# 2InfinityN6eyond/AbsoluteTrack

Hardware: AMD Instinct MI355X
Metric: hand-frames/sec (higher is better)
Workload: dtype f32 (backbone products as two fp16 pieces per operand, fp32 accumulation); 1 GPU; 4 fisheye cameras x 2 hands per frame, 2 views per hand, 96x96 crops, known-skeleton path, full hot path (resample+backbone+head+FK) + all-gather of records; frames_per_gpu=1024, src_image=480x636 u8 x 4 cameras, parallelism=frame-shard x1, world=1, backend=none (single process), outputs_finite=True

## Files before the change

absolutetrack_amd/csrc/conv_c32s2.hip:

```cpp
#include "ut_kernels.h"
#include "ut_conv_dev.h"

namespace ut {
namespace {

constexpr int S_OPIX = 96;
constexpr int S_PROWS = 432;
constexpr int S_STAGE = S_PROWS * 128;
constexpr int S_ZROW = 2 * S_STAGE;
constexpr int S_W8 = S_ZROW + 256;
constexpr int S_CNT = S_W8 + 2 * 4096;
constexpr int S_LDS = S_CNT + 32;
constexpr unsigned S_HOOB = 0x80000000u;
static_assert(S_ZROW % 256 == 0, "zero block bank-row aligned");

#define UT_AR_TAP_8 "v", "v", "v", "v"

}

__global__ __launch_bounds__(512, 1) void conv_c32s2_kernel(Stride2Launch p, int n_tiles) {
  extern __shared__ __attribute__((aligned(16))) char smem[];
  const unsigned smem_addr = (unsigned)(unsigned long)(lds_char*)smem;
  const int tid = threadIdx.x;
  const int lane = tid & 63;
  const int wave = __builtin_amdgcn_readfirstlane(tid >> 6);
  const bool mfma_wave = wave < 6;
  const int cb = wave & 1;
  const int blk = mfma_wave ? wave >> 1 : 0;
  const int fr = lane & 31, fh = lane >> 5;
  const int W = p.W, Wo = p.W / 2;
  const int tiles_per_img = p.H / 8;
  const int M_in = p.n_img * p.H * p.W;
  const int M_out = p.n_img * (p.H / 2) * Wo;
  constexpr int CIN = 32, COUT = 64;

  float x_scale = 1.f, x_unscale = 1.f;
  if (p.in_max) {
    bool ok, adapted;
    split_act_scale(p.in_max, p.in_obs, p.split_adaptive, x_scale, x_unscale, ok, adapted);
    split_scale_report(ok, adapted, p.status, p.adapt_count);
  }
  const float unscale1 = p.unscale1 * x_unscale, unscale_d = p.unscale_d * x_unscale;

  const u32x4 a_words = rsrc_words(p.in, (unsigned)((size_t)M_in * CIN * sizeof(float)));
  const __amdgpu_buffer_rsrc_t o1_rsrc = __builtin_amdgcn_make_buffer_rsrc(p.out1, 0, (int)((size_t)M_out * COUT * sizeof(float)), 0x00020000);
  const __amdgpu_buffer_rsrc_t o2_rsrc = __builtin_amdgcn_make_buffer_rsrc(p.out2, 0, (int)((size_t)M_out * COUT * sizeof(float)), 0x00020000);

  u32x4 wa[32], wd[4];
  {
    const char* wg = reinterpret_cast<const char*>(p.w1_split) + (size_t)cb * 9 * 4096 + lane * 16;
    asm volatile(
        "global_load_dwordx4 %0, %16, off offset:0\n\t"
        "global_load_dwordx4 %1, %16, off offset:1024\n\t"
        "global_load_dwordx4 %2, %16, off offset:2048\n\t"
        "global_load_dwordx4 %3, %16, off offset:3072\n\t"
        "global_load_dwordx4 %4, %17, off offset:0\n\t"
        "global_load_dwordx4 %5, %17, off offset:1024\n\t"
        "global_load_dwordx4 %6, %17, off offset:2048\n\t"
        "global_load_dwordx4 %7, %17, off offset:3072\n\t"
        "global_load_dwordx4 %8, %18, off offset:0\n\t"
        "global_load_dwordx4 %9, %18, off offset:1024\n\t"
        "global_load_dwordx4 %10, %18, off offset:2048\n\t"
        "global_load_dwordx4 %11, %18, off offset:3072\n\t"
        "global_load_dwordx4 %12, %19, off offset:0\n\t"
        "global_load_dwordx4 %13, %19, off offset:1024\n\t"
        "global_load_dwordx4 %14, %19, off offset:2048\n\t"
        "global_load_dwordx4 %15, %19, off offset:3072\n\t"
        "s_waitcnt vmcnt(0)"
        : "=&" UT_ARF_0(wa[0]), "=&" UT_ARF_1(wa[1]), "=&" UT_ARF_2(wa[2]), "=&" UT_ARF_3(wa[3]), "=&" UT_ARF_4(wa[4]), "=&" UT_ARF_5(wa[5]), "=&" UT_ARF_6(wa[6]), "=&" UT_ARF_7(wa[7]), "=&" UT_ARF_8(wa[8]), "=&" UT_ARF_9(wa[9]), "=&" UT_ARF_10(wa[10]), "=&" UT_ARF_11(wa[11]), "=&" UT_ARF_12(wa[12]), "=&" UT_ARF_13(wa[13]), "=&" UT_ARF_14(wa[14]), "=&" UT_ARF_15(wa[15])
        : "v"(wg + 0 * 4096), "v"(wg + 1 * 4096), "v"(wg + 2 * 4096), "v"(wg + 3 * 4096)
        : "memory");
    asm volatile(
        "global_load_dwordx4 %0, %16, off offset:0\n\t"
        "global_load_dwordx4 %1, %16, off offset:1024\n\t"
        "global_load_dwordx4 %2, %16, off offset:2048\n\t"
        "global_load_dwordx4 %3, %16, off offset:3072\n\t"
        "global_load_dwordx4 %4, %17, off offset:0\n\t"
        "global_load_dwordx4 %5, %17, off offset:1024\n\t"
        "global_load_dwordx4 %6, %17, off offset:2048\n\t"
        "global_load_dwordx4 %7, %17, off offset:3072\n\t"
        "global_load_dwordx4 %8, %18, off offset:0\n\t"
        "global_load_dwordx4 %9, %18, off offset:1024\n\t"
        "global_load_dwordx4 %10, %18, off offset:2048\n\t"
        "global_load_dwordx4 %11, %18, off offset:3072\n\t"
        "global_load_dwordx4 %12, %19, off offset:0\n\t"
        "global_load_dwordx4 %13, %19, off offset:1024\n\t"
        "global_load_dwordx4 %14, %19, off offset:2048\n\t"
        "global_load_dwordx4 %15, %19, off offset:3072\n\t"
        "s_waitcnt vmcnt(0)"
        : "=&" UT_ARF_16(wa[16]), "=&" UT_ARF_17(wa[17]), "=&" UT_ARF_18(wa[18]), "=&" UT_ARF_19(wa[19]), "=&" UT_ARF_20(wa[20]), "=&" UT_ARF_21(wa[21]), "=&" UT_ARF_22(wa[22]), "=&" UT_ARF_23(wa[23]), "=&" UT_ARF_24(wa[24]), "=&" UT_ARF_25(wa[25]), "=&" UT_ARF_26(wa[26]), "=&" UT_ARF_27(wa[27]), "=&" UT_ARF_28(wa[28]), "=&" UT_ARF_29(wa[29]), "=&" UT_ARF_30(wa[30]), "=&" UT_ARF_31(wa[31])
        : "v"(wg + 4 * 4096), "v"(wg + 5 * 4096), "v"(wg + 6 * 4096), "v"(wg + 7 * 4096)
        : "memory");
    if (wave < 2) {
#pragma unroll
      for (int q = 0; q < 4; ++q)
        *reinterpret_cast<u32x4*>(smem + S_W8 + cb * 4096 + q * 1024 + lane * 16) = *reinterpret_cast<const u32x4*>(wg + 8 * 4096 + q * 1024);
    }
    const char* dg = reinterpret_cast<const char*>(p.wd_split) + (size_t)cb * 4096 + lane * 16;
#pragma unroll
    for (int q = 0; q < 4; ++q) wd[q] = *reinterpret_cast<const u32x4*>(dg + q * 1024);
  }
  const unsigned w8 = (unsigned)(S_W8 + cb * 4096 + lane * 16);

  if (tid < 16) *reinterpret_cast<u32x4*>(smem + S_ZROW + tid * 16) = u32x4{0, 0, 0, 0};
  if (tid == 16) *reinterpret_cast<u32x4*>(smem + S_CNT) = u32x4{0, 0, 0, 0};

  const int grid = gridDim.x;
  const int my_tiles = (n_tiles - (int)blockIdx.x + grid - 1) / grid;
  const int n_pieces = (9 * W + 7) / 8;
  int lane_o = lane, wave_o = wave;
  auto patch_first_pixel = [&](int tile) {
    const int img = tile / tiles_per_img, q = tile - img * tiles_per_img;
    return img * p.H * W + (8 * q - 1) * W;
  };
  auto issue_patch_piece = [&](int i, int first_pixel, int buf) {
    const int q = wave_o + 8 * i;
    if (q < n_pieces) {
      const int pos = 8 * q + (lane_o >> 3);
      const int row = (pos & ~3) | ((pos & 1) << 1) | ((pos >> 1) & 1);
      const int pix = first_pixel + row;
      const bool ok = pix >= 0 && pix < M_in && row < 9 * W;
      const unsigned off = ok ? (unsigned)(pix * CIN + 4 * ((lane_o & 7) ^ ((row >> 2) & 7))) * 4u : S_HOOB;
      dma_piece(a_words, (unsigned)__builtin_amdgcn_readfirstlane((int)(smem_addr + (unsigned)(buf * S_STAGE + q * 1024))), off, 0u);
    }
  };
  auto convert_row = [&](int buf, int row) {
    const int sw = (row >> 2) & 7;
    char* rp = smem + buf * S_STAGE + row * 128;
    float4 f[8];
#pragma unroll
    for (int g4 = 0; g4 < 8; ++g4) f[g4] = *reinterpret_cast<const float4*>(rp + ((g4 ^ sw) << 4));
#pragma unroll
    for (int kg = 0; kg < 4; ++kg) {
      unsigned a0, a1, a2, a3, b0, b1, b2, b3;
      split_pair_scaled(f[2 * kg].x, f[2 * kg].y, x_scale, a0, b0);
      split_pair_scaled(f[2 * kg].z, f[2 * kg].w, x_scale, a1, b1);
      split_pair_scaled(f[2 * kg + 1].x, f[2 * kg + 1].y, x_scale, a2, b2);
      split_pair_scaled(f[2 * kg + 1].z, f[2 * kg + 1].w, x_scale, a3, b3);
      u32x4 a, b;
      a.x = a0; a.y = a1; a.z = a2; a.w = a3;
      b.x = b0; b.y = b1; b.z = b2; b.w = b3;
      *reinterpret_cast<u32x4*>(rp + ((kg ^ sw) << 4)) = a;
      *reinterpret_cast<u32x4*>(rp + (((4 + kg) ^ sw) << 4)) = b;
    }
  };
  auto unit_pos = [&](int u) { return (u & ~31) | (4 * ((u & 15) >> 1) + (u & 1) + 2 * ((u >> 4) & 1)); };
  auto convert_share = [&](int buf) {
    int t_ = tid;
    asm volatile("" : "+v"(t_));
    if (t_ >= 384) {
      convert_row(buf, unit_pos(t_ - 384));
      convert_row(buf, unit_pos(t_ - 384 + 128));
    } else {
      const int pos = unit_pos(256 + t_);
      if (256 + t_ < ((9 * W + 31) & ~31) && pos < 9 * W) convert_row(buf, pos);
    }
  };

  {
    const int fp = patch_first_pixel((int)blockIdx.x);
#pragma unroll
    for (int i = 0; i < 7; ++i) issue_patch_piece(i, fp, 0);
  }
  asm volatile("s_waitcnt vmcnt(0) lgkmcnt(0)" ::: "memory");
  __syncthreads();
  convert_share(0);
  __builtin_amdgcn_s_waitcnt(0xC07F);
  __builtin_amdgcn_s_barrier();

  unsigned out_bits = 0;
  const float bias1 = p.bias1[32 * cb + fr], bias_d = p.bias_d[32 * cb + fr];
  const int o_ = 32 * blk + fr, oy_ = o_ / Wo, ox_ = o_ - oy_ * Wo;
  const int lrow = 2 * oy_ * W + 2 * ox_ - 1;
  const unsigned mask_left = ox_ == 0 ? 0x1FFu & ~0x49u : 0x1FFu;
  const unsigned mask_top = oy_ == 0 ? 0x1FFu & ~0x7u : 0x1FFu;
  const unsigned cnt_addr = smem_addr + (unsigned)S_CNT;

#define S_PIN() __builtin_amdgcn_sched_barrier(0)
#define S_SIGNAL(ADDR)                                                                               \
  {                                                                                                  \
    unsigned long long keep_;                                                                        \
    asm volatile("s_mov_b64 %0, exec\n\ts_mov_b64 exec, 1\n\tds_add_u32 %1, %2\n\ts_mov_b64 exec, %0" \
                 : "=&s"(keep_) : "v"(ADDR), "v"(1u) : "memory");                                    \
  }
#define S_AWAIT(ADDR, TARGET)                                                                        \
  for (;;) {                                                                                         \
    unsigned seen_;                                                                                  \
    asm volatile("ds_read_b32 %0, %1\n\ts_waitcnt lgkmcnt(0)" : "=v"(seen_) : "v"(ADDR) : "memory"); \
    if ((int)(__builtin_amdgcn_readfirstlane(seen_) - (unsigned)(TARGET)) >= 0) break;               \
    __builtin_amdgcn_s_sleep(1);                                                                     \
  }
#define S_MFMA_A(ACC, TAP, S, PL, PXV) asm volatile("v_mfma_f32_32x32x16_f16 %0, %1, %2, %0" : "+v"(ACC) : "v"(PXV), UT_AR(TAP, S, PL)(wa[S_W(TAP, S, PL)]))
#define S_MFMA_A_FIRST(ACC, TAP, S, PL, PXV) asm volatile("s_nop 3\n\tv_mfma_f32_32x32x16_f16 %0, %1, %2, %0" : "+v"(ACC) : "v"(PXV), UT_AR(TAP, S, PL)(wa[S_W(TAP, S, PL)]))
#define S_MFMA_V(ACC, WV, PXV) asm volatile("v_mfma_f32_32x32x16_f16 %0, %1, %2, %0" : "+v"(ACC) : "v"(PXV), "v"(WV))
#define S_MFMA_V_FIRST(ACC, WV, PXV) asm volatile("s_nop 3\n\tv_mfma_f32_32x32x16_f16 %0, %1, %2, %0" : "+v"(ACC) : "v"(PXV), "v"(WV))
#define S_MFMA_V_LAST(ACC, WV, PXV) asm volatile("v_mfma_f32_32x32x16_f16 %0, %1, %2, %0\n\ts_nop 15\n\ts_nop 7" : "+v"(ACC) : "v"(PXV), "v"(WV))
#define S_W(TAP, S, PL) (((TAP) * 4 + (S) * 2 + (PL)) & 31)
#define S_ADDR(DST, BUF, TAP)                                                                        \
  {                                                                                                  \
    const int row_ = lrow_t + ((TAP) / 3) * W + ((TAP) % 3);                                         \
    const int pos_ = (row_ & ~3) | ((row_ & 1) << 1) | ((row_ >> 1) & 1);                            \
    const unsigned a_ = (unsigned)(BUF) + (unsigned)(pos_ * 128) + (unsigned)(((fh ^ ((row_ >> 2) & 7))) << 4); \
    DST = ((rmask >> (TAP)) & 1u) ? a_ : (unsigned)S_ZROW + (a_ & 255u);                             \
  }
#define S_LOAD(DST, ADDR, S)                                                                         \
  {                                                                                                  \
    DST[0] = *reinterpret_cast<const u32x4*>(smem + ((ADDR) ^ (32u * (S))));                         \
    DST[1] = *reinterpret_cast<const u32x4*>(smem + ((ADDR) ^ (32u * (S)) ^ 64u));                   \
  }
#define S_STEP(TAP, S, CUR, FAR, PIECE, ADN, ADF)                                                    \
  {                                                                                                  \
    u32x4 w8a_, w8b_;                                                                                \
    if constexpr ((TAP) == 8) {                                                                      \
      w8a_ = *reinterpret_cast<const u32x4*>(smem + w8 + ((S) * 2 + 0) * 1024);                      \
      w8b_ = *reinterpret_cast<const u32x4*>(smem + w8 + ((S) * 2 + 1) * 1024);                      \
    }                                                                                                \
    if constexpr ((TAP) < 8) {                                                                       \
      if constexpr ((TAP) == 0 && (S) == 0) { S_MFMA_A_FIRST(acc, TAP, S, 0, CUR[1]); } else { S_MFMA_A(acc, TAP, S, 0, CUR[1]); } \
    } else { S_MFMA_V(acc, w8a_, CUR[1]); }                                                          \
    S_PIN();                                                                                         \
    if constexpr ((TAP) < 8) S_LOAD(FAR, ADN, S);                                                    \
    S_PIN();                                                                                         \
    if constexpr ((TAP) < 8) { S_MFMA_A(acc, TAP, S, 1, CUR[0]); } else { S_MFMA_V(acc, w8b_, CUR[0]); } \
    S_PIN();                                                                                         \
    if constexpr ((S) == 1 && (TAP) < 7) S_ADDR(ADF, rbuf, (TAP) + 2);                               \
    S_PIN();                                                                                         \
    if constexpr ((TAP) < 8) { S_MFMA_A(acc, TAP, S, 0, CUR[0]); }                                   \
    else if constexpr ((S) == 1) { S_MFMA_V_LAST(acc, w8a_, CUR[0]); } else { S_MFMA_V(acc, w8a_, CUR[0]); } \
    S_PIN();                                                                                         \
    if constexpr ((TAP) == 4) {                     \
      if constexpr ((S) == 0) { S_MFMA_V_FIRST(accd, wd[0], CUR[1]); } else { S_MFMA_V(accd, wd[2], CUR[1]); } \
      S_PIN();                                                                                       \
      S_MFMA_V(accd, wd[2 * (S) + 1], CUR[0]); S_PIN();                                              \
      if constexpr ((S) == 1) { S_MFMA_V_LAST(accd, wd[2], CUR[0]); } else { S_MFMA_V(accd, wd[0], CUR[0]); } \
      S_PIN();                                                                                       \
    }                                                                                                \
    if ((PIECE) < 7 && dma_on) issue_patch_piece(PIECE, f_first, f_buf);                             \
    if ((PIECE) == 77 && dma_on) {       \
      asm volatile("s_waitcnt vmcnt(0)" ::: "memory");                      \
      S_SIGNAL(cnt_addr);                                                                            \
    }                                                                                                \
    S_PIN();                                                                                         \
  }

#define S_ROFF(OFF, R) ((((R) >> 3) ? (OFF) + 16u * COUT * 4u : (OFF)) + (unsigned)(((((R) >> 2) & 1) * 8 + ((R) & 3)) * COUT * 4))
#define S_EPILOGUE()                                                                                 \
  {                                                                                                  \
    const unsigned off = (unsigned)((tile * S_OPIX + 32 * blk + 4 * fh) * COUT + 32 * cb + fr) * 4u; \
    unsigned mx = 0;                                                                                 \
    _Pragma("unroll") for (int r = 0; r < 16; ++r) {                                                 \
      const float o = fmaxf(__builtin_fmaf(acc[r], unscale1, bias1), 0.f);                           \
      mx = max(mx, __float_as_uint(o));                                                              \
      __builtin_amdgcn_raw_buffer_store_b32(__float_as_uint(o), o1_rsrc, S_ROFF(off, r), 0, 0);      \
    }                                                                                                \
    out_bits = max(out_bits, mx);                                                                    \
    _Pragma("unroll") for (int r = 0; r < 16; ++r) {                                                 \
      const float o = __builtin_fmaf(accd[r], unscale_d, bias_d);                                    \
      __builtin_amdgcn_raw_buffer_store_b32(__float_as_uint(o), o2_rsrc, S_ROFF(off, r), 0, 0);      \
    }                                                                                                \
  }

  f32x16 acc, accd;
  for (int k = 0; k < my_tiles; ++k) {
    const int tile = blockIdx.x + k * grid;
    const unsigned rbuf = (unsigned)((k & 1) * S_STAGE);
    const bool dma_on = k + 1 < my_tiles;
    const int f_buf = (k + 1) & 1;
    const int f_first = patch_first_pixel(tile + grid);
    asm volatile("" : "+v"(lane_o));
    asm volatile("" : "+s"(wave_o));
    if (mfma_wave) {
      const int tq = tile % tiles_per_img;
      const unsigned rmask = mask_left & (tq == 0 ? mask_top : 0x1FFu);
      int lrow_t = lrow;
      asm volatile("" : "+v"(lrow_t));
#pragma unroll
      for (int e = 0; e < 16; ++e) { acc[e] = 0.f; accd[e] = 0.f; }
      asm volatile("" : "+v"(acc), "+v"(accd));
      {
        u32x4 pxA[2], pxB[2], pxC[2];
        unsigned adE, adO;
        S_ADDR(adE, rbuf, 0);
        S_LOAD(pxA, adE, 0);
        S_LOAD(pxB, adE, 1);
        S_ADDR(adO, rbuf, 1);
        S_STEP(0, 0, pxA, pxC, 0, adO, adE)   S_STEP(0, 1, pxB, pxA, 1, adO, adE)
        S_STEP(1, 0, pxC, pxB, 2, adE, adO)   S_STEP(1, 1, pxA, pxC, 3, adE, adO)
        S_STEP(2, 0, pxB, pxA, 4, adO, adE)   S_STEP(2, 1, pxC, pxB, 5, adO, adE)
        S_STEP(3, 0, pxA, pxC, 6, adE, adO)   S_STEP(3, 1, pxB, pxA, 99, adE, adO)
        S_STEP(4, 0, pxC, pxB, 99, adO, adE)  S_STEP(4, 1, pxA, pxC, 99, adO, adE)
        S_STEP(5, 0, pxB, pxA, 99, adE, adO)  S_STEP(5, 1, pxC, pxB, 99, adE, adO)
        S_STEP(6, 0, pxA, pxC, 99, adO, adE)  S_STEP(6, 1, pxB, pxA, 99, adO, adE)
        S_STEP(7, 0, pxC, pxB, 77, adE, adO)  S_STEP(7, 1, pxA, pxC, 99, adE, adO)
        S_STEP(8, 0, pxB, pxA, 99, adO, adE)  S_STEP(8, 1, pxC, pxB, 99, adO, adE)
      }
      asm volatile("s_nop 15\n\ts_nop 3" : "+v"(acc), "+v"(accd));
      if (wave >= 4) S_EPILOGUE();
    } else if (dma_on) {
#pragma unroll
      for (int i = 0; i < 7; ++i) issue_patch_piece(i, f_first, f_buf);
      asm volatile("s_waitcnt vmcnt(0)" ::: "memory");
      S_SIGNAL(cnt_addr);
    }
    if (dma_on) {
      S_AWAIT(cnt_addr, 8 * (k + 1))
      convert_share(f_buf);
    }
    asm volatile("s_waitcnt lgkmcnt(0)" ::: "memory");
    __builtin_amdgcn_s_barrier();
    if (mfma_wave && wave < 4) S_EPILOGUE();
  }
  asm volatile("s_waitcnt vmcnt(0)" ::: "memory");
  if (p.out1_max) publish_abs_max(p.out1_max, out_bits);
#undef S_PIN
#undef S_SIGNAL
#undef S_AWAIT
#undef S_MFMA_A
#undef S_MFMA_A_FIRST
#undef S_MFMA_V
#undef S_MFMA_V_FIRST
#undef S_MFMA_V_LAST
#undef S_W
#undef S_ADDR
#undef S_LOAD
#undef S_STEP
#undef S_EPILOGUE
#undef S_ROFF
}

bool conv_c32s2_applicable(const Stride2Launch& c) {
  return c.in && c.out1 && c.out2 && c.w1_split && c.wd_split && c.unscale1 > 0.f && c.unscale_d > 0.f && c.in_max && c.W == 48 &&
         c.H % 8 == 0 && c.H >= 8 && c.n_img > 0 && c.num_cu > 0 && (size_t)c.n_img * c.H * c.W * 32 * sizeof(float) < 0x7FFFFF00ull;
}

hipError_t launch_conv_c32s2(const Stride2Launch& c, hipStream_t s) {
  if (!conv_c32s2_applicable(c)) return hipErrorInvalidValue;
  const int n_tiles = c.n_img * (c.H / 8);
  static std::atomic<unsigned long long> attr_set{0};
  const hipError_t attr_e = set_dynamic_lds_once(attr_set, c.device, S_LDS, &conv_c32s2_kernel);
  if (attr_e != hipSuccess) return attr_e;
  int grid = c.num_cu;
  if (grid > n_tiles) grid = n_tiles;
  hipLaunchKernelGGL(conv_c32s2_kernel, dim3(grid), dim3(512), S_LDS, s, c, n_tiles);
  return hipGetLastError();
}

}
```

absolutetrack_amd/csrc/conv_split.hip:

```cpp
#include <math.h>

#include "ut_kernels.h"
#include "ut_conv_dev.h"

namespace ut {
namespace {

typedef __attribute__((address_space(3))) unsigned lds_u32;

constexpr unsigned OOB = 0xFFFFFF00u;

__device__ __forceinline__ int fdiv(int n, int d, float inv_d) {
  int q = (int)((float)n * inv_d);
  int r = n - q * d;
  if (r < 0) --q;
  if (r >= d) ++q;
  return q;
}

__device__ __forceinline__ f16x8 frag(const unsigned (&v)[4]) {
  u32x4 t;
  t.x = v[0]; t.y = v[1]; t.z = v[2]; t.w = v[3];
  return __builtin_bit_cast(f16x8, t);
}
// ... 250 lines not shown
    acc[i_][j_] = __builtin_amdgcn_mfma_f32_32x32x16_f16(frag(xp[SET][i_][xp_]), frag(wf[SET][j_][wp_]), acc[i_][j_], 0, 0, 0); \
  }

#define SP_SIGNAL(ADDR, LGKM)                                                                         \
  {                                                                                                  \
    unsigned long long keep_;                                                                        \
    if constexpr (LGKM) asm volatile("s_waitcnt lgkmcnt(0)" ::: "memory");                           \
    asm volatile("s_mov_b64 %0, exec\n\ts_mov_b64 exec, 1\n\tds_add_u32 %1, %2\n\ts_mov_b64 exec, %0" \
                 : "=&s"(keep_) : "v"(ADDR), "v"(1u) : "memory");                                    \
  }
                                                                     \
#define SP_PEEK(ADDR) (*reinterpret_cast<volatile lds_u32*>(ADDR))
#define SP_AWAIT(PEEKED, ADDR, TARGET)                                                               \
  if ((int)(__builtin_amdgcn_readfirstlane(PEEKED) - (TARGET)) < 0) {                                \
    for (;;) {                                                                                       \
      unsigned seen_;                                                                                \
      asm volatile("ds_read_b32 %0, %1\n\ts_waitcnt lgkmcnt(0)" : "=v"(seen_) : "v"(ADDR) : "memory"); \
      if ((int)(__builtin_amdgcn_readfirstlane(seen_) - (TARGET)) >= 0) break;                       \
    }                                                                                                \
  }
#define SP_SLOT(CUR, NXT, N, FIRST)                                                                  \
  {                                                                                                  \
    if constexpr (FIRST && (N) == 0) {                                                               \
                                        \
      if (skip_waits > 0) --skip_waits;                                                              \
      else if constexpr (!HALO) asm volatile("s_waitcnt vmcnt(%0)" ::"n"(WP + AP) : "memory");       \
      else if (prev_had_patch) asm volatile("s_waitcnt vmcnt(%0)" ::"n"(WP + 1) : "memory");         \
      else asm volatile("s_waitcnt vmcnt(%0)" ::"n"(WP) : "memory");                                 \
      SP_SIGNAL(landed_addr, 0);                                                                              \
    }                                                                                                \
     \
    if constexpr (!HALO && FIRST && (N) == ARR) SP_SIGNAL(read_addr, 1);          \
    if constexpr (!HALO && (FIRST ? 0 : NM) + (N) == RW - PEEK) read_seen = SP_PEEK(read_addr);       \
    if constexpr (FIRST && (N) == NM - PEEK) landed_seen = SP_PEEK(landed_addr);                     \
    if constexpr (!FIRST && NM + (N) == RW) {                                                        \
      if constexpr (!HALO) {                                                                         \
        read_target += 8u;                                                                           \
        SP_AWAIT(read_seen, read_addr, read_target);                                                 \
      }                                                                                              \
          \
      if (c == 1 && tid == 0) {                                                                      \
        int t_ = ticket;                                                                             \
        asm volatile("" : "+v"(t_));    \
        slot_write(slot_addr, grid + t_);                                                            \
      }                                                                                              \
    }                                                                                                \
                    \
    constexpr int g_ = (FIRST ? 0 : NM) + (N) - PS0;                                                 \
    if constexpr (g_ >= 0 && g_ % PSTEP == 0 && g_ / PSTEP < WP) SP_W_ISSUE(g_ / PSTEP);              \
    if constexpr (!HALO && g_ >= 0 && g_ % PSTEP == 0 && g_ / PSTEP >= WP && g_ / PSTEP < WP + AP) SP_A_ADDR(g_ / PSTEP - WP, a_off); \
    if constexpr (!HALO && g_ >= ASEP && (g_ - ASEP) % PSTEP == 0 && (g_ - ASEP) / PSTEP >= WP && (g_ - ASEP) / PSTEP < WP + AP) \
      SP_A_ISSUE((g_ - ASEP) / PSTEP - WP, a_off);                                                   \
    if constexpr (HALO && g_ == WP * PSTEP) {       \
      if (c_tap == 0) SP_H_ISSUE(0, f_slice);                                                        \
      else if (c_tap == 1) SP_H_ISSUE(1, f_slice);                                                   \
      else if (c_tap == 2) SP_H_ISSUE(2, f_slice);                                                   \
      else if (c_tap == 3) SP_H_ISSUE(3, f_slice);                                                   \
      else if (c_tap == 4) SP_H_ISSUE(4, f_slice);                                                   \
    }                                                                                                \
    if constexpr (!HALO && (N) >= CV0 && (N) - CV0 < UNITS) SP_CONV(NXT, (N) - CV0);                 \
    if constexpr ((N) >= RD0 && (N) - RD0 < NWF) SP_READ_W1(NXT, FIRST ? 1 : 0, (N) - RD0);          \
    SP_PIN();                                                                                        \
    SP_MFMA(CUR, N);                                                                                 \
    SP_PIN();                                                                                        \
  }
#define SP_SLOTS3(CUR, NXT, N, FIRST) SP_SLOT(CUR, NXT, N, FIRST) SP_SLOT(CUR, NXT, (N) + 1, FIRST) SP_SLOT(CUR, NXT, (N) + 2, FIRST)
#define SP_STEP(CUR, NXT, FIRST)                                                                     \
  {                                                                                                  \
    __builtin_amdgcn_s_setprio(2);                                                                   \
    SP_SLOTS3(CUR, NXT, 0, FIRST) SP_SLOTS3(CUR, NXT, 3, FIRST)                                      \
    if constexpr (NM > 6) { SP_SLOTS3(CUR, NXT, 6, FIRST) SP_SLOTS3(CUR, NXT, 9, FIRST) }            \
    __builtin_amdgcn_s_setprio(0);                                                                   \
  }
  static_assert(NM == 6 || NM == 12, "SP_STEP expands 6 or 12 slots");
  static_assert(NPH == 5, "SP_SLOT issues patch pieces 0..4");

  const unsigned slot_addr = smem_addr + (unsigned)SLOT;
  const unsigned read_addr = slot_addr + 4, landed_addr = slot_addr + 8;
  unsigned read_target = 0, landed_target = 0, read_seen = 0, landed_seen = 0;
  if (tid == 0) asm volatile("ds_write_b32 %0, %1\n\tds_write_b32 %2, %1" ::"v"(read_addr), "v"(0u), "v"(landed_addr) : "memory");
  if constexpr (!HALO) SP_A_SETUP();
  SP_W_SETUP();
  unsigned a_off = 0;
  int skip_waits = 0;
  bool prev_had_patch = false;
  int f_slice = 0;
  if (lane < 16 && wave == 0) asm volatile("ds_write_b128 %0, %1" ::"v"(smem_addr + (unsigned)ZROW + (unsigned)lane * 16u), "v"(u32x4{0, 0, 0, 0}) : "memory");
  if constexpr (HALO) {
    SP_H_SETUP(slot);
    SP_H_MASK(slot);
    SP_H_ISSUE(0, 0); SP_H_ISSUE(1, 0); SP_H_ISSUE(2, 0); SP_H_ISSUE(3, 0); SP_H_ISSUE(4, 0);
    h_buf = A_STAGE;
    f_slice = n_slices > 1 ? 1 : 0;
  }
#pragma unroll
  for (int c = 0; c < W_AHEAD; ++c) {
    if constexpr (!HALO) {
      SP_A_TAP();
#pragma unroll
      for (int i = 0; i < AP; ++i) { SP_A_ADDR(i, a_off); SP_A_ISSUE(i, a_off); }
      SP_A_ADVANCE();
    }
#pragma unroll
    for (int t = 0; t < WP; ++t) SP_W_ISSUE(t);
    SP_W_ADVANCE();
  }
  asm volatile("s_waitcnt vmcnt(0) lgkmcnt(0)" ::: "memory");
  __syncthreads();
#pragma unroll
  for (int i = 0; i < MI; ++i)
#pragma unroll
    for (int j = 0; j < NI; ++j)
#pragma unroll
      for (int e = 0; e < 16; ++e) acc[i][j][e] = 0.f;
  if constexpr (HALO) {
    SP_H_CONVERT(0u);
    asm volatile("s_waitcnt lgkmcnt(0)" ::: "memory");
    __syncthreads();
  }
  SP_READ_X(0, 0u);
  SP_READ_WALL(0, 0);
  if constexpr (!HALO) {
    SP_CONV(0, 0) SP_CONV(0, 1) SP_CONV(0, 2) SP_CONV(0, 3)
    if constexpr (UNITS > 4) { SP_CONV(0, 4) SP_CONV(0, 5) SP_CONV(0, 6) SP_CONV(0, 7) }
  }

  constexpr bool EARLY_RES = MI * NI <= 2;
#define SP_PIX(I, R) (wm * (MI * 32) + (I) * 32 + 8 * ((R) >> 2) + 4 * fh + ((R) & 3))
#define SP_BASE(TM, TN, J) ((TN) * BN + wn * (NI * 32) + (J) * 32 + fr < p.cout_store                   \
                                ? (unsigned)(((TM) * BM + wm * (MI * 32) + 4 * fh) * p.cout_store + (TN) * BN + wn * (NI * 32) + (J) * 32 + fr) * 4u \
                                : HOOB)
  float rr[MI][NI][16];
#define SP_RES_REQUEST()                                                                             \
  {                                                                                                  \
    const int tm_ = tile / tiles_n, tn_ = tile - tm_ * tiles_n;                                      \
    const unsigned row_b_ = (unsigned)p.cout_store * 4u;                                             \
    _Pragma("unroll") for (int j = 0; j < NI; ++j) {                                                 \
      unsigned off_ = SP_BASE(tm_, tn_, j);                                                          \
      _Pragma("unroll") for (int i = 0; i < MI; ++i)                                                 \
        _Pragma("unroll") for (int r = 0; r < 16; ++r) {                                             \
          rr[i][j][r] = __uint_as_float(__builtin_amdgcn_raw_buffer_load_b32(r_rsrc, off_, 0, 0));   \
          off_ += ((r & 3) == 3 ? 5u : 1u) * row_b_;       \
        }                                                                                            \
    }                                                                                                \
  }
  unsigned out_bits = 0;
  int tile = slot;
  for (;;) {
    const int ticket = __builtin_amdgcn_raw_ptr_buffer_atomic_add_i32(1, q_rsrc, q_off, 0, 0);
    for (int c = 0; c < n_chunks; ++c) {
      if (c == n_chunks - (HALO ? 9 : 3)) {
        int nv;
        asm volatile("ds_read_b32 %0, %1\n\ts_waitcnt lgkmcnt(0)" : "=v"(nv) : "v"(slot_addr) : "memory");
        next_tile = __builtin_amdgcn_readfirstlane(nv);
        if constexpr (HALO) {
          SP_H_SETUP(next_tile);
          f_slice = 0;
        } else {
          fa_tile = next_tile;
          SP_A_SETUP();
        }
      }
      if (c == n_chunks - W_AHEAD) {
        fw_tile = next_tile;
        SP_W_SETUP();
      }
      if constexpr (!HALO) SP_A_TAP();
      if constexpr (EARLY_RES) {
        if (c == n_chunks - 1) SP_RES_REQUEST();
      }
      SP_READ_X(1, rd_a);
      SP_STEP(0, 1, true)
      rd_a = rd_a + A_STAGE == A_RING * A_STAGE ? 0u : rd_a + A_STAGE;
      rd_w = rd_w + W_STAGE == W_RING * W_STAGE ? 0u : rd_w + W_STAGE;
      if constexpr (HALO) {
        if (++r_tap == 9) {
          r_tap = 0;
          r_buf ^= (unsigned)A_STAGE;
          if (c == n_chunks - 1) SP_H_MASK(next_tile);
        }
      }
      landed_target += 8u;
      SP_AWAIT(landed_seen, landed_addr, landed_target);
      if constexpr (HALO) {
        if (c_tap == 7) {
          SP_H_CONVERT(h_buf);
          asm volatile("s_waitcnt lgkmcnt(0)" ::: "memory");
        }
      }
      SP_READ_X(0, rd_a);
      SP_STEP(1, 0, false)
      if constexpr (HALO) {
        prev_had_patch = c_tap < NPH;
        if (++c_tap == 9) {
          c_tap = 0;
          h_buf ^= (unsigned)A_STAGE;
          ++c_slice;
          if (c_slice == n_slices) c_slice = 0;
          f_slice = c_slice + 1 < n_slices ? c_slice + 1 : 0;
        }
      } else {
        SP_A_ADVANCE();
      }
      SP_W_ADVANCE();
    }
    {
      const int tm = tile / tiles_n, tn = tile - tm * tiles_n;
      const float floor_v = p.relu ? 0.f : -__builtin_huge_valf();
      float bb[NI];
#pragma unroll
      for (int j = 0; j < NI; ++j) bb[j] = p.bias[tn * BN + wn * (NI * 32) + j * 32 + fr];
      if constexpr (!EARLY_RES) SP_RES_REQUEST();
      if constexpr (EARLY_RES) asm volatile("s_waitcnt vmcnt(0)" ::: "memory");
      const unsigned row_b = (unsigned)p.cout_store * 4u;
      const bool ragged = tm * BM + BM > M;
#pragma unroll
      for (int j = 0; j < NI; ++j) {
        unsigned off = SP_BASE(tm, tn, j);
        const unsigned keep_n = off != HOOB ? 0x7FFFFFFFu : 0u;
#pragma unroll
        for (int i = 0; i < MI; ++i) {
#pragma unroll
          for (int r = 0; r < 16; ++r) {
            const unsigned o = __float_as_uint(fmaxf(fmaf(acc[i][j][r], tot_unscale, bb[j] + rr[i][j][r]), floor_v));
            const unsigned keep = ragged ? (tm * BM + SP_PIX(i, r) < M ? keep_n : 0u) : keep_n;
            out_bits = max(out_bits, o & keep);
            __builtin_amdgcn_raw_buffer_store_b32(o, o_rsrc, off, 0, 0);
            off += ((r & 3) == 3 ? 5u : 1u) * row_b;
          }
#pragma unroll
          for (int e = 0; e < 16; ++e) acc[i][j][e] = 0.f;
        }
      }
      skip_waits = 2;
    }
    if ((unsigned)next_tile >= (unsigned)n_tiles) break;
    tile = next_tile;
  }
  asm volatile("s_waitcnt vmcnt(0)" ::: "memory");
  if (p.out_max) publish_abs_max(p.out_max, out_bits);
#undef SP_H_SETUP
#undef SP_H_ISSUE
#undef SP_H_MASK
#undef SP_H_CONVERT
#undef SP_A_SETUP
#undef SP_W_SETUP
#undef SP_A_TAP
#undef SP_A_ADDR
#undef SP_A_ISSUE
#undef SP_A_ADVANCE
#undef SP_W_ISSUE
#undef SP_W_ADVANCE
#undef SP_READ_X
#undef SP_READ_WALL
#undef SP_READ_W1
#undef SP_CONV
#undef SP_PIN
#undef SP_MFMA
#undef SP_SLOT
#undef SP_RES_REQUEST
#undef SP_PIX
#undef SP_BASE
#undef SP_SIGNAL
#undef SP_AWAIT
#undef SP_PEEK
#undef SP_SLOTS3
#undef SP_STEP
}

template <int BM, int BN, int WR, int WC, bool HALO>
hipError_t launch_split_cfg(const ConvLaunch& c, hipStream_t s) {
  const int M = c.n_img * c.Ho * c.Wo;
  const int tiles_m = (M + BM - 1) / BM;
  const int tiles_n = (c.cout_store + BN - 1) / BN;
  const int n_tiles = tiles_m * tiles_n;
  const size_t lds = (HALO ? 2 * (size_t)320 * 128 : 3 * (size_t)BM * 128) + (HALO ? 4 : 3) * (size_t)BN * 128 + 256 + 16;
  static std::atomic<unsigned long long> attr_set{0};
  const hipError_t attr_e = set_dynamic_lds_once(attr_set, c.device, (int)lds, &conv_split_kernel<BM, BN, WR, WC, HALO>);
  if (attr_e != hipSuccess) return attr_e;
  int grid = c.num_cu;
  if (grid > n_tiles) grid = n_tiles;
  hipLaunchKernelGGL((conv_split_kernel<BM, BN, WR, WC, HALO>), dim3(grid), dim3(512), lds, s, c, tiles_n, n_tiles);
  return hipGetLastError();
}

}

bool conv_split_applicable(const ConvLaunch& c) {
  return c.w_split && c.split_unscale > 0.f && c.cslice == 32 && c.cin % 32 == 0 && !c.out_nchw && c.splits == 0 && c.k_pad / 32 >= 6 &&
         c.cout_store % 4 == 0 && c.cout_store >= 64 && c.tile_counter && c.num_cu > 0;
}

hipError_t launch_conv_split(const ConvLaunch& c, hipStream_t s) {
  if (!conv_split_applicable(c)) return hipErrorInvalidValue;
  if ((size_t)c.n_img * c.H * c.W * c.cin * sizeof(float) >= 0x7FFFFF00ull) return hipErrorInvalidValue;
  if ((size_t)c.n_img * c.Ho * c.Wo * c.cout_store * sizeof(float) >= 0x7FFFFF00ull) return hipErrorInvalidValue;
  if (conv_w4_applicable(c)) return launch_conv_w4(c, s);
  if (conv_c64k_applicable(c)) return launch_conv_c64k(c, s);
  const bool halo = c.ksize == 3 && c.stride == 1 && c.pad == 1 && c.cin >= 64 && c.W <= 31 && c.H == c.Ho && c.W == c.Wo;
  if (c.cout_store <= 64) return halo ? launch_split_cfg<256, 64, 8, 1, true>(c, s) : launch_split_cfg<256, 64, 8, 1, false>(c, s);
  return halo ? launch_split_cfg<256, 128, 4, 2, true>(c, s) : launch_split_cfg<256, 128, 4, 2, false>(c, s);
}

size_t pack_split_weights(const float* w, int cout_pad, int k_pad, float scale, uint16_t* out) {
  const int n_chunks = k_pad / 32;
  for (int grp = 0; grp < cout_pad / 32; ++grp)
    for (int kc = 0; kc < n_chunks; ++kc)
      for (int st = 0; st < 2; ++st)
        for (int ln = 0; ln < 64; ++ln)
          for (int e = 0; e < 8; ++e) {
            const float x = w[(size_t)(grp * 32 + (ln & 31)) * k_pad + kc * 32 + 16 * st + 8 * (ln >> 5) + e] * scale;
            const _Float16 h0 = (_Float16)x;
            const _Float16 h1 = (_Float16)(x - (float)h0);
            const size_t base = ((((size_t)grp * n_chunks + kc) * 2 + st) * 2) * 512 + (size_t)ln * 8 + e;
            __builtin_memcpy(&out[base], &h0, 2);
            __builtin_memcpy(&out[base + 512], &h1, 2);
          }
  return (size_t)2 * cout_pad * k_pad;
}

float split_weight_scale(const float* w, size_t n) {
  float m = 0.f;
  for (size_t i = 0; i < n; ++i) m = fmaxf(m, fabsf(w[i]));
  if (!(m > 0.f) || !(m < 3.0e38f)) return 1.f;
  int e;
  frexpf(m, &e);
  return ldexpf(1.f, 15 - e);
}

}
```

absolutetrack_amd/csrc/conv_w4.hip:

```cpp
#include "ut_kernels.h"
#include "ut_conv_dev.h"

namespace ut {
namespace {

constexpr int W4_WPIX = 288;
constexpr int W4_MI = 9;
constexpr int W4_NLOAD = 9;
constexpr int W4_NSTG = 5;
constexpr int W4_DIST = 2;
constexpr int W4_NSET = W4_DIST + 1;
constexpr unsigned W4_HOOB = 0x80000000u;
static_assert(9 % W4_NSET == 0, "the register sets of the weight fragments line up across slices");
constexpr int w4_cap(int pixels, int wi, int hi) { return ((pixels / (wi * hi)) * (hi + 1) * (wi + 1) + 2 * (wi + 2) + 15) / 16 * 16; }

template <int WI, int HI, int SCH, int WPX, bool S2 = false>
__global__ __launch_bounds__(256, 1) void conv_w4_kernel(ConvLaunch p, int tiles_n, int n_tiles) {
  extern __shared__ __attribute__((aligned(16))) char smem[];
  constexpr int MI = W4_MI, PW = WI + 1, PH = HI + 1, HW = WI * HI;
  static_assert(!S2 || (SCH == 32 && WPX == 1), "phase planes: two 16-channel planes per buffer, four 32-channel blocks per tile");
  constexpr int BM = W4_WPIX * WPX;
  constexpr int NCB = 4 / WPX, BN = 32 * NCB;
  constexpr int NG = SCH / 4, NHG = NG / 2;
  constexpr int KS = 9 * SCH / 16;
  constexpr int NBUF = SCH == 32 ? 2 : 3;
  constexpr int AHEAD = NBUF - 1;
  constexpr int RP = 256 / NG;
  constexpr int CAP = w4_cap(BM, WI, HI);
  constexpr int GSTRIDE = CAP * 16;
  constexpr int STAGE = NG * GSTRIDE;
  constexpr int SLOT = NBUF * STAGE;
  constexpr int EPI = SLOT + 16;
  static_assert(BM % HW == 0, "a tile is a whole number of maps: every tile has the same padded layout");
  static_assert(BM * NG == W4_NLOAD * 256 && KS % W4_NSET == 0 && (SCH == 32 || SCH == 16) && (WPX == 1 || WPX == 2), "shape");
  static_assert((NG - 2) * GSTRIDE + (2 * PW + 2) * 16 < 65536, "fragment reads: everything but the lane's base fits the immediate offset");

  const int tid = threadIdx.x;
  const int lane = tid & 63;
  const int wave = __builtin_amdgcn_readfirstlane(tid >> 6);
  const int wm = WPX == 1 ? 0 : wave >> 1;
  const int wco = WPX == 1 ? wave : wave & 1;
  const int fr = lane & 31, fh = lane >> 5;

  const int M = p.n_img * HW;
  const int n_slices = p.cin / (S2 ? 16 : SCH);
  const int n_chunks = p.k_pad / 32;

  const __amdgpu_buffer_rsrc_t a_rsrc = __builtin_amdgcn_make_buffer_rsrc(
      const_cast<float*>(p.in), 0, (int)((size_t)M * (S2 ? 4 : 1) * p.cin * sizeof(float)), 0x00020000);
  const __amdgpu_buffer_rsrc_t w_rsrc = __builtin_amdgcn_make_buffer_rsrc(
      const_cast<void*>(p.w_split), 0, (int)((size_t)(p.cout_pad / 32) * n_chunks * 4096), 0x00020000);
  const __amdgpu_buffer_rsrc_t r_rsrc = __builtin_amdgcn_make_buffer_rsrc(
      const_cast<float*>(p.res ? p.res : p.bias), 0, p.res ? (int)((size_t)M * p.cout_store * sizeof(float)) : 0, 0x00020000);
  const __amdgpu_buffer_rsrc_t o_rsrc =
      __builtin_amdgcn_make_buffer_rsrc(p.out, 0, (int)((size_t)M * p.cout_store * sizeof(float)), 0x00020000);
  const __amdgpu_buffer_rsrc_t q_rsrc = __builtin_amdgcn_make_buffer_rsrc(p.tile_counter, 0, 4, 0x00020000);

  float x_scale = 1.f, x_unscale = 1.f;
  if (p.in_max) {
    bool ok, adapted;
    split_act_scale(p.in_max, p.in_obs, p.split_adaptive, x_scale, x_unscale, ok, adapted);
    split_scale_report(ok, adapted, p.status, p.adapt_count);
  }
  const float tot_unscale = p.split_unscale * x_unscale;
  const float floor_v = p.relu ? 0.f : -__builtin_huge_valf();
  const unsigned row_b = (unsigned)p.cout_store * 4u;

  const int grid = gridDim.x;
  int slot = blockIdx.x;
  if ((grid & 7) == 0) slot = (blockIdx.x & 7) * (grid >> 3) + (blockIdx.x >> 3);

  unsigned h_wa[W4_NLOAD], pb[MI];
#pragma unroll
  for (int j = 0; j < W4_NLOAD; ++j) {
    const int k = RP * j + tid / NG, img = k / HW, rem = k - img * HW, y = rem / WI, x = rem - y * WI;
    h_wa[j] = (unsigned)((PW + 1 + img * (PH * PW) + y * PW + x) * 16 + ((tid % NG) >> 1) * GSTRIDE + (tid & 1) * 8);
  }
#pragma unroll
  for (int i = 0; i < MI; ++i) {
    const int k = wm * W4_WPIX + 32 * i + fr, img = k / HW, rem = k - img * HW, y = rem / WI, x = rem - y * WI;
    pb[i] = (unsigned)((img * (PH * PW) + y * PW + x) * 16 + fh * GSTRIDE);
  }
  const unsigned h_step = (unsigned)(RP * p.cin) * 4u;
#define W4_H_BASE(TILE) ((unsigned)((((TILE) / tiles_n) * BM + tid / NG) * p.cin + 4 * (tid % NG)) * 4u)
  unsigned h_in[S2 ? W4_NLOAD : 1], po_a = 0, po_b = 0, pb1[S2 ? MI : 1];
  if constexpr (S2) {
#pragma unroll
    for (int j = 0; j < W4_NLOAD; ++j) {
      const int k = RP * j + tid / NG, img = k / HW, rem = k - img * HW, y = rem / WI, x = rem - y * WI;
      h_in[j] = (unsigned)(((img * 2 * HI + 2 * y) * 2 * WI + 2 * x) * p.cin + 4 * (tid & 3)) * 4u;
    }
    const bool second = (tid & 4) != 0;
    po_a = second ? 0u : (unsigned)((2 * WI + 1) * p.cin) * 4u;
    po_b = second ? (unsigned)(2 * WI * p.cin) * 4u : (unsigned)p.cin * 4u;
#pragma unroll
    for (int i = 0; i < MI; ++i) pb1[i] = pb[i] + (unsigned)STAGE;
  }
#define W4S_BASE(TILE) ((unsigned)(((TILE) / tiles_n) * (BM * 4)) * (unsigned)p.cin * 4u)

  f32x16 acc[MI];
  u32x4 xp[MI][2];
  u32x4 wf[W4_NSET][2];
  float4 stg[S2 ? W4_NLOAD : W4_NSTG];
  const unsigned w_lane = (unsigned)lane * 16u;

#define W4_READ_X(I, PC, S, TAP, BASE)                                                               \
  xp[I][PC] = *reinterpret_cast<const u32x4*>(smem + (BASE)[I] + (unsigned)(((PC) * NHG + (SCH == 32 ? 2 * (S) : 0)) * GSTRIDE + (((TAP) / 3) * PW + (TAP) % 3) * 16));
#define W4_LOAD_W(SET, PL, CH, S, WROW)                                                              \
  {                                                                                                  \
    const unsigned so_ = (WROW) + (unsigned)((wco * n_chunks + (CH)) * 4096 + ((S) * 2 + (PL)) * 1024); \
    wf[SET][PL] = __builtin_bit_cast(u32x4, __builtin_amdgcn_raw_buffer_load_b128(w_rsrc, w_lane, so_, 0)); \
  }
#define W4S_PLANE(Q) ((0x190 >> (Q)) & 1)
#define W4S_TAPP(Q) ((int)((0x414344310ull >> (4 * (Q))) & 15))
#define W4S_TAPO(Q) ((int)((0x715348620ull >> (4 * (Q))) & 15))
#define W4S_BASEOF(Q) ((Q) >= 5 ? pb1 : pb)
#define W4_TAP(Q) (SCH == 32 ? (Q) >> 1 : (Q))
#define W4_CHUNK(SL, Q) (SCH == 32 ? (SL) * 9 + ((Q) >> 1) : ((SL) >> 1) * 9 + (Q))
#define W4_HALF(SL, Q) (SCH == 32 ? (Q) & 1 : (SL) & 1)
#define W4_MFMA(WSET, N)                                                                             \
  {                                                                                                  \
    constexpr int pr_ = (N) / MI, i_ = (N) % MI;                                                     \
    constexpr int wp_ = pr_ == 1 ? 1 : 0, xq_ = pr_ == 0 ? 1 : 0;       \
    acc[i_] = __builtin_amdgcn_mfma_f32_32x32x16_f16(__builtin_bit_cast(f16x8, xp[i_][xq_]),         \
                                                     __builtin_bit_cast(f16x8, wf[WSET][wp_]), acc[i_], 0, 0, 0);  \
  }
#define W4_PIN() { __builtin_amdgcn_sched_barrier(0); asm volatile("" ::: "memory"); __builtin_amdgcn_sched_barrier(0); }
#define W4_ROW_OFF(I, R) ((unsigned)((I) * 32 + 8 * ((R) >> 2) + ((R) & 3)) * row_bs)
#define W4_SPLIT_STORE(V, WA)                                                                        \
  {                                                                                                  \
    unsigned a0_, b0_, a1_, b1_;                                                                     \
    split_pair_scaled((V).x, (V).y, x_scale, a0_, b0_);                                              \
    split_pair_scaled((V).z, (V).w, x_scale, a1_, b1_);                                              \
    *reinterpret_cast<u32x2*>(smem + (WA)) = u32x2{a0_, a1_};                                        \
    *reinterpret_cast<u32x2*>(smem + (WA) + NHG * GSTRIDE) = u32x2{b0_, b1_};                        \
  }

  int tile = slot;
  int next_tile = 0;
  int cur_buf = 0;
  unsigned out_bits = 0;
  const unsigned slot_addr = (unsigned)(unsigned long)(lds_char*)smem + (unsigned)SLOT;

  for (int k = tid; k < NBUF * STAGE / 16; k += 256) *reinterpret_cast<u32x4*>(smem + k * 16) = u32x4{0, 0, 0, 0};
  __syncthreads();
  unsigned h_base = S2 ? 0u : W4_H_BASE(tile);
  unsigned w_row = (unsigned)((tile % tiles_n) * NCB) * (unsigned)n_chunks * 4096u;
  unsigned w_row_next = w_row;
  if constexpr (!S2) {
#pragma unroll
    for (int a = 0; a < AHEAD; ++a)
#pragma unroll
      for (int j = 0; j < W4_NLOAD; ++j) {
        const float4 v = __builtin_bit_cast(float4, __builtin_amdgcn_raw_buffer_load_b128(a_rsrc, h_base + (unsigned)j * h_step, (unsigned)(a * SCH * 4), 0));
        if (a == AHEAD - 1 && KS == 9 && j >= W4_NLOAD - 4) stg[j % W4_NSTG] = v;
        else W4_SPLIT_STORE(v, (unsigned)(a * STAGE) + h_wa[j])
      }
#pragma unroll
    for (int g = 0; g < W4_DIST; ++g) { W4_LOAD_W(g, 0, W4_CHUNK(0, g), W4_HALF(0, g), w_row) W4_LOAD_W(g, 1, W4_CHUNK(0, g), W4_HALF(0, g), w_row) }
  } else {
    const unsigned t0 = W4S_BASE(tile);
#pragma unroll
    for (int j = 0; j < W4_NLOAD; ++j) {
      const float4 v = __builtin_bit_cast(float4, __builtin_amdgcn_raw_buffer_load_b128(a_rsrc, h_in[j] + po_a + t0, 0, 0));
      W4_SPLIT_STORE(v, h_wa[j])
    }
#pragma unroll
    for (int j = 0; j < W4_NLOAD; ++j) {
      const float4 v = __builtin_bit_cast(float4, __builtin_amdgcn_raw_buffer_load_b128(a_rsrc, h_in[j] + po_b + t0, 0, 0));
      if (j == 0) W4_SPLIT_STORE(v, (unsigned)STAGE + h_wa[j])
      else stg[j] = v;
    }
#pragma unroll
    for (int g = 0; g < W4_DIST; ++g) { W4_LOAD_W(g, 0, W4S_TAPO(g), 0, w_row) W4_LOAD_W(g, 1, W4S_TAPO(g), 0, w_row) }
  }
  __syncthreads();
#pragma unroll
  for (int i = 0; i < MI; ++i) {
    W4_READ_X(i, 1, 0, 0, pb)
    if (i < MI - 1) { W4_READ_X(i, 0, 0, 0, pb) }
  }

#define W4_SLOT_BODY(N)                                                                              \
        {                                                                                            \
          if ((N) == 0 && q != KS - 1) { W4_READ_X(MI - 1, 0, W4_HALF(sl, q), W4_TAP(q), rb) }       \
          if ((N) >= 1 && (N) <= 9 && q1 < KS) { W4_READ_X(((N) + 8) % 9, 1, W4_HALF(sl, q1), W4_TAP(q1), rb) } \
          if ((N) >= 1 && (N) <= 9 && q1 == KS) { W4_READ_X(((N) + 8) % 9, 1, 0, 0, nb) }            \
          if ((N) >= 19 && (N) <= 26 && q1 < KS) { W4_READ_X(((N) + 8) % 9, 0, W4_HALF(sl, q1), W4_TAP(q1), rb) } \
          if ((N) >= 19 && (N) <= 26 && q1 == KS) { W4_READ_X(((N) + 8) % 9, 0, 0, 0, nb) }          \
          if (((N) == 10 || (N) == 11) && qd < KS) { W4_LOAD_W(qd % W4_NSET, (N) & 1, W4_CHUNK(sl, qd), W4_HALF(sl, qd), w_row) } \
          if (((N) == 10 || (N) == 11) && qd >= KS) { W4_LOAD_W(qd % W4_NSET, (N) & 1, W4_CHUNK(sl_after, qd - KS), W4_HALF(sl_after, qd - KS), row_after) } \
          if ((N) == 12 && q >= 4 && q < 4 + W4_NLOAD) { const float4 v_ = stg[(q + W4_NSTG - 4) % W4_NSTG]; split_pair_scaled(v_.x, v_.y, x_scale, cv0, cv1); } \
          if ((N) == 13 && q >= 4 && q < 4 + W4_NLOAD) {                                             \
            const float4 v_ = stg[(q + W4_NSTG - 4) % W4_NSTG];                                      \
            unsigned a1_, b1_;                                                                       \
            split_pair_scaled(v_.z, v_.w, x_scale, a1_, b1_);                                        \
            *reinterpret_cast<u32x2*>(smem + wbuf + h_wa[(q + 5) % 9]) = u32x2{cv0, a1_};            \
            *reinterpret_cast<u32x2*>(smem + wbuf + h_wa[(q + 5) % 9] + NHG * GSTRIDE) = u32x2{cv1, b1_}; \
          }                                                                                          \
          if (KS == 9 && (N) == 12 && q < 4) { const float4 v_ = stg[q % W4_NSTG]; split_pair_scaled(v_.x, v_.y, x_scale, cv0, cv1); } \
          if (KS == 9 && (N) == 13 && q < 4) {       \
            const float4 v_ = stg[q % W4_NSTG];                                                      \
            unsigned a1_, b1_;                                                                       \
            split_pair_scaled(v_.z, v_.w, x_scale, a1_, b1_);                                        \
            *reinterpret_cast<u32x2*>(smem + pbuf + h_wa[q + 5]) = u32x2{cv0, a1_};                  \
            *reinterpret_cast<u32x2*>(smem + pbuf + h_wa[q + 5] + NHG * GSTRIDE) = u32x2{cv1, b1_};  \
          }                                                                                          \
          if ((N) == 14 && q < W4_NLOAD)                                                             \
            stg[q % W4_NSTG] = __builtin_bit_cast(float4, __builtin_amdgcn_raw_buffer_load_b128(a_rsrc, h_base + (unsigned)q * h_step, f_soff, 0)); \
          if ((N) == 16 && q == KS / 2 && sl == 0 && tid == 0) *reinterpret_cast<int*>(smem + SLOT) = grid + ticket; \
          W4_PIN();                                                                                  \
          W4_MFMA(ws, N);                                                                            \
          W4_PIN();                                                                                  \
        }
#define W4_SLICE()                                                                                   \
      _Pragma("clang loop unroll(full)") for (int q = 0; q < KS; ++q) {                              \
        const int ws = q % W4_NSET;                                                                  \
        unsigned cv0 = 0, cv1 = 0;      \
         \
        const int q1 = q + 1, qd = q + W4_DIST;                                                      \
        if (q == KS - 1) {                                                                           \
                                       \
          W4_READ_X(MI - 1, 0, W4_HALF(sl, KS - 1), 8, rb)                                           \
          asm volatile("s_waitcnt lgkmcnt(0)" ::: "memory");                                         \
          __builtin_amdgcn_s_barrier();                                                              \
          asm volatile("" ::: "memory");                                                             \
          if (sl == 0) {                                                                             \
            next_tile = slot_read(slot_addr);                                                        \
            w_row_next = (unsigned)((next_tile % tiles_n) * NCB) * (unsigned)n_chunks * 4096u;       \
          }                                                                                          \
        }                                                                                            \
        W4_SLOT_BODY(0) W4_SLOT_BODY(1) W4_SLOT_BODY(2) W4_SLOT_BODY(3) W4_SLOT_BODY(4) W4_SLOT_BODY(5) W4_SLOT_BODY(6) W4_SLOT_BODY(7) W4_SLOT_BODY(8) \
        W4_SLOT_BODY(9) W4_SLOT_BODY(10) W4_SLOT_BODY(11) W4_SLOT_BODY(12) W4_SLOT_BODY(13) W4_SLOT_BODY(14) W4_SLOT_BODY(15) W4_SLOT_BODY(16) W4_SLOT_BODY(17) \
        W4_SLOT_BODY(18) W4_SLOT_BODY(19) W4_SLOT_BODY(20) W4_SLOT_BODY(21) W4_SLOT_BODY(22) W4_SLOT_BODY(23) W4_SLOT_BODY(24) W4_SLOT_BODY(25) W4_SLOT_BODY(26) \
      }

#define W4S_CV_N(Q) ((Q) == 4 ? 3 : (Q) == 8 ? 1 : 2)
#define W4S_CV_J(Q, NN) ((Q) < 4 ? 2 * (Q) + 1 + (NN) : (Q) == 4 ? (NN) : (Q) < 8 ? 2 * (Q) - 7 + (NN) : 0)
#define W4S_CV_DST(Q) (((Q) < 4 || (Q) == 8) ? (unsigned)STAGE : 0u)
#define W4S_LD_N(Q) ((Q) == 0 ? 3 : (Q) == 4 ? 1 : 2)
#define W4S_LD_J(Q, NN) ((Q) == 0 ? (NN) : (Q) < 4 ? 2 * (Q) + 1 + (NN) : (Q) == 4 ? 0 : 2 * (Q) - 9 + (NN))
#define W4S_SLOT_BODY(N)                                                                             \
        {                                                                                            \
          if ((N) == 0) { W4_READ_X(MI - 1, 0, W4S_PLANE(q), W4S_TAPP(q), W4S_BASEOF(q)) }          \
          if ((N) == 9 && (q == 4 || q == 8)) {                                                      \
                                         \
            asm volatile("s_waitcnt lgkmcnt(0)" ::: "memory");                                       \
            __builtin_amdgcn_s_barrier();                                                            \
            asm volatile("" ::: "memory");                                                           \
            if (q == 8 && sl == 0) {                                                                 \
              next_tile = slot_read(slot_addr);                                                      \
              w_row_next = (unsigned)((next_tile % tiles_n) * NCB) * (unsigned)n_chunks * 4096u;     \
            }                                                                                        \
          }                                                                                          \
          if ((N) >= 1 && (N) <= 9 && q != 4 && q != 8) { W4_READ_X(((N) + 8) % 9, 1, W4S_PLANE(q1), W4S_TAPP(q1), W4S_BASEOF(q1)) } \
          if ((N) >= 10 && (N) <= 18 && (q == 4 || q == 8)) { W4_READ_X(((N) + 8) % 9, 1, W4S_PLANE(q1), W4S_TAPP(q1), W4S_BASEOF(q1)) } \
          if ((N) >= 19 && (N) <= 26) { W4_READ_X(((N) + 8) % 9, 0, W4S_PLANE(q1), W4S_TAPP(q1), W4S_BASEOF(q1)) } \
          if (((N) == 10 || (N) == 11) && qd < 9) { W4_LOAD_W(qd % W4_NSET, (N) & 1, (sl >> 1) * 9 + W4S_TAPO(qd), sl & 1, w_row) } \
          if (((N) == 10 || (N) == 11) && qd >= 9) { W4_LOAD_W(qd % W4_NSET, (N) & 1, (sl_after >> 1) * 9 + W4S_TAPO(qd - 9), sl_after & 1, row_after) } \
           \
          if ((N) >= 10 && (N) <= 21 && ((N) - 10) / 4 < W4S_CV_N(q)) {                              \
            const float4 v_ = stg[W4S_CV_J(q, ((N) - 10) / 4) % 9];                                  \
            constexpr int part_ = ((N) - 10) & 3;                                                    \
            if (part_ == 0 || part_ == 2) {                                                          \
              const f16x2 h_ = __builtin_bit_cast(f16x2, __builtin_amdgcn_cvt_pkrtz((part_ ? v_.z : v_.x) * x_scale, (part_ ? v_.w : v_.y) * x_scale)); \
              (part_ ? cvh1 : cvh0) = __builtin_bit_cast(unsigned, h_);                              \
              cvf = (float)h_[0];                                                                    \
            } else {                                                                                 \
              const f16x2 h_ = __builtin_bit_cast(f16x2, part_ == 1 ? cvh0 : cvh1);                  \
              const float ra_ = __builtin_fmaf(part_ == 1 ? v_.x : v_.z, x_scale, -cvf);             \
              const float rb_ = __builtin_fmaf(part_ == 1 ? v_.y : v_.w, x_scale, -(float)h_[1]);    \
              const unsigned p_ = __builtin_bit_cast(unsigned, __builtin_amdgcn_cvt_pkrtz(ra_, rb_)); \
              if (part_ == 1) cvp0 = p_;                                                             \
              else {                                                                                 \
                *reinterpret_cast<u32x2*>(smem + W4S_CV_DST(q) + h_wa[W4S_CV_J(q, ((N) - 10) / 4) % 9]) = u32x2{cvh0, cvh1}; \
                *reinterpret_cast<u32x2*>(smem + W4S_CV_DST(q) + h_wa[W4S_CV_J(q, ((N) - 10) / 4) % 9] + NHG * GSTRIDE) = u32x2{cvp0, p_}; \
              }                                                                                      \
            }                                                                                        \
          }                                                                                          \
          if ((N) >= 22 && (N) <= 24 && (N) - 22 < W4S_LD_N(q))                                      \
            stg[W4S_LD_J(q, (N) - 22) % 9] = __builtin_bit_cast(float4, __builtin_amdgcn_raw_buffer_load_b128(    \
                a_rsrc, h_in[W4S_LD_J(q, (N) - 22) % 9] + (q < 4 ? hb_a : hb_b), f_soff, 0));        \
          if ((N) == 16 && q == 1 && sl == 0 && tid == 0) *reinterpret_cast<int*>(smem + SLOT) = grid + ticket; \
          W4_PIN();                                                                                  \
          W4_MFMA(ws, N);                                                                            \
          W4_PIN();                                                                                  \
        }
#define W4S_SLICE()                                                                                  \
      _Pragma("clang loop unroll(full)") for (int q = 0; q < 9; ++q) {                               \
        const int ws = q % W4_NSET;                                                                  \
        unsigned cvh0 = 0, cvh1 = 0, cvp0 = 0;                       \
        float cvf = 0.f;                                                                             \
        const int q1 = (q + 1) % 9, qd = q + W4_DIST;                                                \
        W4S_SLOT_BODY(0) W4S_SLOT_BODY(1) W4S_SLOT_BODY(2) W4S_SLOT_BODY(3) W4S_SLOT_BODY(4) W4S_SLOT_BODY(5) W4S_SLOT_BODY(6) W4S_SLOT_BODY(7) W4S_SLOT_BODY(8) \
        W4S_SLOT_BODY(9) W4S_SLOT_BODY(10) W4S_SLOT_BODY(11) W4S_SLOT_BODY(12) W4S_SLOT_BODY(13) W4S_SLOT_BODY(14) W4S_SLOT_BODY(15) W4S_SLOT_BODY(16) W4S_SLOT_BODY(17) \
        W4S_SLOT_BODY(18) W4S_SLOT_BODY(19) W4S_SLOT_BODY(20) W4S_SLOT_BODY(21) W4S_SLOT_BODY(22) W4S_SLOT_BODY(23) W4S_SLOT_BODY(24) W4S_SLOT_BODY(25) W4S_SLOT_BODY(26) \
      }

  for (;;) {
    int ticket = 0;
    if (tid == 0) ticket = __builtin_amdgcn_raw_ptr_buffer_atomic_add_i32(1, q_rsrc, 0, 0, 0);
#pragma unroll
    for (int i = 0; i < MI; ++i)
#pragma unroll
      for (int e = 0; e < 16; ++e) acc[i][e] = 0.f;

    const float4 bb4 = *reinterpret_cast<const float4*>(p.bias + (tile % tiles_n) * BN + wco * 32 + 4 * (lane & 7));
    if constexpr (S2) {
      for (int sl = 0; sl < n_slices; ++sl) {
        const bool last_slice = sl == n_slices - 1;
        const unsigned f_soff = last_slice ? 0u : (unsigned)(sl + 1) * 64u;
        const unsigned f_tb = W4S_BASE(last_slice ? next_tile : tile);
        const unsigned hb_a = po_a + f_tb, hb_b = po_b + f_tb;
        const int sl_after = last_slice ? 0 : sl + 1;
        const unsigned row_after = last_slice ? w_row_next : w_row;
        W4S_SLICE()
      }
    } else
    for (int sl = 0; sl < n_slices; ++sl) {
      const bool last_slice = sl == n_slices - 1;
      const int b1 = cur_buf + 1 == NBUF ? 0 : cur_buf + 1, b2 = b1 + 1 == NBUF ? 0 : b1 + 1;
      unsigned rbuf = (unsigned)__builtin_amdgcn_readfirstlane(cur_buf * STAGE), nbuf = (unsigned)__builtin_amdgcn_readfirstlane(b1 * STAGE);
      unsigned wbuf = (unsigned)__builtin_amdgcn_readfirstlane((NBUF == 2 ? b1 : b2) * STAGE), pbuf = nbuf;
      asm volatile("" : "+s"(rbuf), "+s"(nbuf), "+s"(wbuf), "+s"(pbuf));
      const int f_sl = sl + AHEAD < n_slices ? sl + AHEAD : sl + AHEAD - n_slices;
      if (sl + AHEAD == n_slices) h_base = W4_H_BASE(next_tile);
      const unsigned f_soff = (unsigned)f_sl * (SCH * 4);
      const int sl_after = last_slice ? 0 : sl + 1;
      const unsigned row_after = last_slice ? w_row_next : w_row;
      unsigned rb[MI], nb[MI];
#pragma unroll
      for (int i = 0; i < MI; ++i) { rb[i] = pb[i] + rbuf; nb[i] = pb[i] + nbuf; }
      W4_SLICE()
      cur_buf = b1;
    }
    {
      const int tm = tile / tiles_n, tn = tile - tm * tiles_n;
      const bool ragged = tm * BM + BM > M;
      const int ch = tn * BN + wco * 32 + fr;
      const float bb = p.bias[ch];
      const unsigned base = ch < p.cout_store ? (unsigned)((tm * BM + wm * W4_WPIX + 4 * fh) * p.cout_store + ch) * 4u : W4_HOOB;
      const unsigned keep_n = base != W4_HOOB ? 0x7FFFFFFFu : 0u;
      if (!ragged) {
        unsigned row_bs = (unsigned)__builtin_amdgcn_readfirstlane((int)row_b);
        asm volatile("" : "+s"(row_bs));
        const int ch4 = tn * BN + wco * 32 + 4 * (lane & 7);
        const unsigned base4 = ch4 < p.cout_store ? (unsigned)((tm * BM + wm * W4_WPIX + (lane >> 3)) * p.cout_store + ch4) * 4u : W4_HOOB;
        const unsigned keep4 = base4 != W4_HOOB ? 0x7FFFFFFFu : 0u;
        float4 rr[S2 ? 1 : 6][4];
        if constexpr (!S2) {
#pragma unroll
          for (int i = 0; i < 5; ++i)
#pragma unroll
            for (int t = 0; t < 4; ++t)
              rr[i][t] = __builtin_bit_cast(float4, __builtin_amdgcn_raw_buffer_load_b128(r_rsrc, base4, (unsigned)(32 * i + 8 * t) * row_bs, 0));
        }
        char* const ex = smem + EPI + wave * 4096;
#define W4_EX_WRITE(H)                                                                               \
        _Pragma("unroll") for (int r = 0; r < 8; ++r)                                                \
          *reinterpret_cast<float*>(ex + ((H) & 1) * 2048 + (8 * (r >> 2) + 4 * fh + (r & 3)) * 128 + fr * 4) = acc[(H) >> 1][8 * ((H) & 1) + r];
        W4_EX_WRITE(0)
#pragma unroll
        for (int h = 0; h < 2 * MI; ++h) {
          const int i = h >> 1;
          if (!S2 && (h & 1) == 0 && i + 5 < MI) {
#pragma unroll
            for (int t = 0; t < 4; ++t)
              rr[(i + 5) % 6][t] = __builtin_bit_cast(float4, __builtin_amdgcn_raw_buffer_load_b128(r_rsrc, base4, (unsigned)(32 * (i + 5) + 8 * t) * row_bs, 0));
          }
          if (h + 1 < 2 * MI) { W4_EX_WRITE(h + 1) }
#pragma unroll
          for (int t2 = 0; t2 < 2; ++t2) {
            const int t = 2 * (h & 1) + t2;
            const float4 a = *reinterpret_cast<const float4*>(ex + (h & 1) * 2048 + (8 * t2 + (lane >> 3)) * 128 + (lane & 7) * 16);
            const float4 res = S2 ? float4{0.f, 0.f, 0.f, 0.f} : rr[S2 ? 0 : i % 6][t];
            u32x4 o;
            o.x = __float_as_uint(fmaxf(fmaf(a.x, tot_unscale, bb4.x + res.x), floor_v));
            o.y = __float_as_uint(fmaxf(fmaf(a.y, tot_unscale, bb4.y + res.y), floor_v));
            o.z = __float_as_uint(fmaxf(fmaf(a.z, tot_unscale, bb4.z + res.z), floor_v));
            o.w = __float_as_uint(fmaxf(fmaf(a.w, tot_unscale, bb4.w + res.w), floor_v));
            unsigned mk;
            asm volatile("v_max3_u32 %0, %2, %3, %4\n\tv_max_u32 %0, %0, %5\n\tv_and_b32 %0, %0, %6\n\tv_max_u32 %1, %1, %0"
                         : "=&v"(mk), "+v"(out_bits) : "v"(o.x), "v"(o.y), "v"(o.z), "v"(o.w), "v"(keep4));
            __builtin_amdgcn_raw_buffer_store_b128(o, o_rsrc, base4, (unsigned)(32 * i + 8 * t) * row_bs, 0);
          }
        }
#undef W4_EX_WRITE
      } else {
#pragma unroll
        for (int i = 0; i < MI; ++i) {
          float r1[16];
          unsigned off = base + (unsigned)(i * 32) * row_b;
#pragma unroll
          for (int r = 0; r < 16; ++r) {
            r1[r] = __uint_as_float(__builtin_amdgcn_raw_buffer_load_b32(r_rsrc, off, 0, 0));
            off += ((r & 3) == 3 ? 5u : 1u) * row_b;
          }
          off = base + (unsigned)(i * 32) * row_b;
#pragma unroll
          for (int r = 0; r < 16; ++r) {
            const unsigned o = __float_as_uint(fmaxf(fmaf(acc[i][r], tot_unscale, bb + r1[r]), floor_v));
            const int pix = wm * W4_WPIX + i * 32 + 8 * (r >> 2) + 4 * fh + (r & 3);
            out_bits = max(out_bits, o & (tm * BM + pix < M ? keep_n : 0u));
            __builtin_amdgcn_raw_buffer_store_b32(o, o_rsrc, off, 0, 0);
            off += ((r & 3) == 3 ? 5u : 1u) * row_b;
          }
        }
      }
    }
    if ((unsigned)next_tile >= (unsigned)n_tiles) break;
    tile = next_tile;
    w_row = w_row_next;
  }
  if (p.out_max) publish_abs_max(p.out_max, out_bits);
#undef W4_H_BASE
#undef W4_READ_X
#undef W4_LOAD_W
#undef W4_TAP
#undef W4_CHUNK
#undef W4_HALF
#undef W4_MFMA
#undef W4_PIN
#undef W4_ROW_OFF
#undef W4_SPLIT_STORE
#undef W4_SLOT_BODY
#undef W4_SLICE
#undef W4S_PLANE
#undef W4S_TAPP
#undef W4S_TAPO
#undef W4S_BASEOF
#undef W4S_BASE
#undef W4S_CV_N
#undef W4S_CV_J
#undef W4S_CV_DST
#undef W4S_LD_N
#undef W4S_LD_J
#undef W4S_SLOT_BODY
#undef W4S_SLICE
}

template <int WI, int HI, int SCH, int WPX, bool S2 = false>
hipError_t launch_w4_cfg(const ConvLaunch& c, hipStream_t s) {
  constexpr int BM = W4_WPIX * WPX, BN = 128 / WPX;
  const long M = (long)c.n_img * c.Ho * c.Wo;
  const int tiles_m = (int)((M + BM - 1) / BM), tiles_n = c.cout_store / BN;
  const int n_tiles = tiles_m * tiles_n;
  constexpr int lds = (SCH == 32 ? 2 : 3) * (SCH / 4) * w4_cap(BM, WI, HI) * 16 + 16 + 4 * 4096;
  static std::atomic<unsigned long long> attr_set{0};
  const hipError_t attr_e = set_dynamic_lds_once(attr_set, c.device, lds, &conv_w4_kernel<WI, HI, SCH, WPX, S2>);
  if (attr_e != hipSuccess) return attr_e;
  int grid = c.num_cu;
  if (grid > n_tiles) grid = n_tiles;
  hipLaunchKernelGGL((conv_w4_kernel<WI, HI, SCH, WPX, S2>), dim3(grid), dim3(256), lds, s, c, tiles_n, n_tiles);
  return hipGetLastError();
}

}

bool conv_w4_applicable(const ConvLaunch& c) {
  const bool common = !(c.no_resident & 2) && c.w_split && c.split_unscale > 0.f && c.ksize == 3 && c.pad == 1 && c.cslice == 32 &&
                      c.cin % 32 == 0 && c.cout_pad >= c.cout_store && !c.out_nchw && c.splits == 0 &&
                      c.k_pad == 9 * c.cin && c.tile_counter && c.num_cu > 0 &&
                      (size_t)c.n_img * c.H * c.W * c.cin * sizeof(float) < 0x7FFFFF00ull &&
                      (size_t)c.n_img * c.Ho * c.Wo * c.cout_store * sizeof(float) < 0x7FFFFF00ull;
  if (!common) return false;
  if (c.stride == 2)
    return !(c.no_resident & 8) && c.cin >= 64  && c.cout_store % 128 == 0 && c.H == 2 * c.Ho && c.W == 2 * c.Wo && !c.res &&
           ((c.Wo == 12 && c.Ho == 12) || (c.Wo == 6 && c.Ho == 6));
  if (c.stride != 1 || c.cin < 64 || c.H != c.Ho || c.W != c.Wo) return false;
  if (c.cout_store % 128 == 0) return (c.W == 12 && c.H == 12) || (c.W == 6 && c.H == 6);
  return !(c.no_resident & 4) && c.cout_store == 64 && c.W == 24 && c.H == 24;
}

hipError_t launch_conv_w4(const ConvLaunch& c, hipStream_t s) {
  if (!conv_w4_applicable(c)) return hipErrorInvalidValue;
  if (c.stride == 2) return c.Wo == 12 ? launch_w4_cfg<12, 12, 32, 1, true>(c, s) : launch_w4_cfg<6, 6, 32, 1, true>(c, s);
  if (c.W == 24) return launch_w4_cfg<24, 24, 16, 2>(c, s);
  return c.W == 12 ? launch_w4_cfg<12, 12, 32, 1>(c, s) : launch_w4_cfg<6, 6, 32, 1>(c, s);
}

}
```

absolutetrack_amd/csrc/ut_api.hip:

```cpp
#include "../../include/umetrack_hip.h"

#include <math.h>
#include <stdio.h>
#include <stdlib.h>
#include <string.h>

#include <cmath>
#include <initializer_list>
#include <mutex>
#include <string>
#include <utility>
#include <vector>

#include "ut_kernels.h"
#include "ut_weights.h"

namespace {

thread_local std::string g_create_error;

struct ConvW : ut::ConvGeom {
  float* w = nullptr;
  void* w_split = nullptr;
  float split_unscale = 0.f;
  float wsum_rows = 0.f;
  float bias_max = 0.f;
  float* bias = nullptr;
};

struct Block {
  ConvW conv1, conv2, ds;
  bool has_ds = false;
};

struct Regressor {
  Block blocks[2];
  Block blocks_split[2];
  float* w_out = nullptr;
  float* b_out = nullptr;
  int c = 0, d = 0;
};

struct ProfEvent { hipEvent_t a, b; double flops;   int kind = 0;
};

}

constexpr int kDefaultChunk = 4096;
constexpr int kMaxChunk = 7281;

struct ut_context {
  int device = 0;
  int num_cu = 256;
  std::string err;
  std::vector<void*> allocs;
  float* stem_w = nullptr; float* stem_b = nullptr;
  Block bb[12];
  ConvW proj, fus0, fus1, fus2, tmp[3];
  float *skel_w = nullptr, *skel_b = nullptr, *skel_scale = nullptr, *skel_shift = nullptr;
  Regressor reg_k, reg_u;
  int chunk = kDefaultChunk;
  size_t ws_crops = 0;
  float *bufX = nullptr, *bufH = nullptr, *bufY = nullptr, *bufD = nullptr;
  size_t crops_ws_floats = 0;
  float* crops_ws = nullptr;
  size_t wsb_crops = 0;
  float *bufL2 = nullptr, *bufP = nullptr, *bufQ = nullptr, *bufBH = nullptr, *bufBD = nullptr;
  size_t ws_samples = 0;
  ut::HeadBuffers hb{};
  size_t ws_skel = 0;
  int slots_cap = 0, slots_used = 0;
  float *mem = nullptr, *prev_ext = nullptr;
  unsigned* counters = nullptr;
  int counter_next = 0;
  unsigned* calib = nullptr;
  unsigned* adapt_count = nullptr;
  int scale_mode = UT_SPLIT_SCALE_CALIBRATED;
  bool calibrated = false;
  bool head_calibrated = false;
  bool calibrating = false;
  unsigned word_gen = 0;
  bool block_fusion = true;
  int resident_weights = 1;
  bool call_split = false;
  int* status = nullptr;
  int* status_host = nullptr;
  int* slot_seen = nullptr;
  int check_mode = UT_CHECK_SYNC;
  int lanes = 1;
  hipStream_t lane_stream[2] = {nullptr, nullptr};
  hipEvent_t ev_fork = nullptr, ev_join[2] = {nullptr, nullptr};
  int conv_arith = UT_CONV_FP32;
  bool latency_mode = false;
  float* splitk_ws = nullptr;
  size_t splitk_floats = 0;
  float* zero_bias = nullptr;
  bool profiling = false;
  std::vector<ProfEvent> prof;
};

namespace {

int fail(ut_handle h, int code, const char* what, hipError_t e = hipSuccess) {
  char buf[512];
  if (e != hipSuccess) snprintf(buf, sizeof buf, "%s: %s", what, hipGetErrorString(e));
  else snprintf(buf, sizeof buf, "%s", what);
  if (h) h->err = buf; else g_create_error = buf;
  return code;
}

#define HIPCHK(h, x)                                            \
  do {                                                          \
    hipError_t e_ = (x);                                        \
    if (e_ != hipSuccess) return fail(h, UT_E_HIP, #x, e_);     \
  } while (0)

struct DeviceScope {
  int prev = -1;
  bool switched = false;
  hipError_t err = hipSuccess;
  explicit DeviceScope(int dev) {
    if (dev < 0) return;
    err = hipGetDevice(&prev);
    if (err == hipSuccess && prev != dev) {
      err = hipSetDevice(dev);
      switched = err == hipSuccess;
    }
  }
  ~DeviceScope() { if (switched) (void)hipSetDevice(prev); }
  DeviceScope(const DeviceScope&) = delete;
  DeviceScope& operator=(const DeviceScope&) = delete;
};
#define ON_DEVICE_IF(h)                                        \
  DeviceScope scope_((h) ? (h)->device : -1);                  \
  if ((h) && scope_.err != hipSuccess) return fail(h, UT_E_HIP, "hipSetDevice", scope_.err)
#define ON_DEVICE_OF(h)                 \
  DeviceScope scope_((h)->device);      \
  if (scope_.err != hipSuccess) return fail(h, UT_E_HIP, "hipSetDevice", scope_.err)

struct DevStatus { int* dev = nullptr; int* host = nullptr; };
std::mutex g_status_mutex;
DevStatus g_status[64];

int stateless_status(int* device_out, DevStatus* out) {
  int dev = 0;
  hipError_t e = hipGetDevice(&dev);
  if (e != hipSuccess) return fail(nullptr, UT_E_HIP, "hipGetDevice", e);
  if (dev < 0 || dev >= 64) return fail(nullptr, UT_E_INVALID, "device index beyond 63");
  std::lock_guard<std::mutex> lock(g_status_mutex);
  DevStatus& st = g_status[dev];
  if (!st.dev) {
    void *d = nullptr, *hst = nullptr;
    if ((e = hipMalloc(&d, 2 * sizeof(int))) != hipSuccess) return fail(nullptr, UT_E_HIP, "hipMalloc", e);
    if ((e = hipHostMalloc(&hst, 2 * sizeof(int), hipHostMallocDefault)) != hipSuccess) {
      (void)hipFree(d);
      return fail(nullptr, UT_E_HIP, "hipHostMalloc", e);
    }
    if ((e = hipMemset(d, 0, 2 * sizeof(int))) != hipSuccess) return fail(nullptr, UT_E_HIP, "hipMemset", e);
    st.dev = (int*)d; st.host = (int*)hst;
  }
  *device_out = dev;
  *out = st;
  return UT_OK;
}

const char* status_message(int bits) {
  if (bits & ut::UT_SPLIT_RANGE)
    return "range check: an activation entering a split-fp16 convolution is an infinity or a NaN, or lies beyond the calibrated range "
           "of its layer (32 x the calibration maximum; ut_calibrate_split with representative crops, UT_SPLIT_SCALE_DYNAMIC or "
           "UT_SPLIT_SCALE_CALIBRATED_ADAPTIVE)";
  if (bits & ut::UT_BAD_SRC_INDEX) return "index check: src_index outside [0, n_src_images)";
  if (bits & ut::UT_BAD_SAMPLE_RANGE) return "index check: sample_range rows must select 1 or 2 crops inside [0, n_crops]";
  if (bits & ut::UT_BAD_MEMORY_IDX) return "index check: memory_idx outside [0, n_slots)";
  if (bits & ut::UT_DUP_MEMORY_IDX) return "index check: memory_idx names one temporal slot twice";
  if (bits & ut::UT_BAD_HAND_IDX) return "index check: hand_idx must be 0 (left) or 1 (right)";
  return "index check: failed";
}

int check_status(ut_handle h, int* dev, int* host, hipStream_t s, const char* what) {
  HIPCHK(h, hipMemcpyAsync(host, dev, 2 * sizeof(int), hipMemcpyDeviceToHost, s));
  HIPCHK(h, hipStreamSynchronize(s));
  const int sticky = host[0];
  if (sticky) HIPCHK(h, hipMemsetAsync(dev, 0, sizeof(int), s));
  if (sticky & ut::UT_STATUS_ERRORS) {
    char buf[256];
    snprintf(buf, sizeof buf, "%s: %s", what, status_message(sticky));
    return fail(h, UT_E_INVALID, buf);
  }
  return UT_OK;
}

int upload_bytes(ut_handle h, const void* host, size_t bytes, void** dev) {
  void* d = nullptr;
  HIPCHK(h, hipMalloc(&d, bytes));
  h->allocs.push_back(d);
  HIPCHK(h, hipMemcpy(d, host, bytes, hipMemcpyHostToDevice));
  *dev = d;
  return UT_OK;
}

int upload(ut_handle h, const std::vector<float>& host, float** dev) {
  return upload_bytes(h, host.data(), host.size() * sizeof(float), (void**)dev);
}

int upload_conv(ut_handle h, ConvW& cw, const ut::PackedConv& pc) {
  static_cast<ut::ConvGeom&>(cw) = pc;
  cw.split_unscale = pc.split_unscale; cw.wsum_rows = pc.wsum_rows; cw.bias_max = pc.bias_max;
  int rc = upload(h, pc.wp, &cw.w);
  if (!rc && !pc.planes.empty()) rc = upload_bytes(h, pc.planes.data(), pc.planes.size() * sizeof(uint16_t), &cw.w_split);
  return rc ? rc : upload(h, pc.bp, &cw.bias);
}

int upload_block(ut_handle h, Block& b, const ut::FoldedBlock& fb) {
  int rc;
  const int cs = ut::round_up(fb.conv1.cout, 4);
  if ((rc = upload_conv(h, b.conv1, ut::pack_conv_host(fb.conv1, 3, fb.stride, cs)))) return rc;
  if ((rc = upload_conv(h, b.conv2, ut::pack_conv_host(fb.conv2, 3, 1, cs)))) return rc;
  b.has_ds = fb.has_ds;
  if (fb.has_ds && (rc = upload_conv(h, b.ds, ut::pack_conv_host(fb.ds, 1, fb.stride, cs)))) return rc;
  return UT_OK;
}

int upload_regressor(ut_handle h, Regressor& r, const ut::FoldedRegressor& fr) {
  r.c = fr.c; r.d = fr.d;
  int rc;
  for (int i = 0; i < 2; ++i)
    if ((rc = upload_block(h, r.blocks[i], fr.blocks[i])) || (rc = upload_block(h, r.blocks_split[i], fr.wide[i]))) return rc;
  if ((rc = upload(h, fr.w_out, &r.w_out))) return rc;
  return upload(h, fr.b_out, &r.b_out);
}

int dev_alloc(ut_handle h, float** p, size_t n_floats) {
  void* d = nullptr;
  HIPCHK(h, hipMalloc(&d, n_floats * sizeof(float)));
  h->allocs.push_back(d);
  *p = (float*)d;
  return UT_OK;
}

void dev_free(ut_handle h, void* p) {
  if (!p) return;
  for (size_t i = 0; i < h->allocs.size(); ++i)
    if (h->allocs[i] == p) { h->allocs.erase(h->allocs.begin() + i); break; }
  (void)hipFree(p);
}

int regrow(ut_handle h, size_t* cap, size_t n, std::initializer_list<std::pair<float**, size_t>> bufs) {
  if (n <= *cap) return UT_OK;
  HIPCHK(h, hipDeviceSynchronize());
  for (auto& b : bufs) { dev_free(h, *b.first); *b.first = nullptr; }
  *cap = 0;
  int rc;
  for (auto& b : bufs)
    if ((rc = dev_alloc(h, b.first, n * b.second))) return rc;
  *cap = n;
  return UT_OK;
}

int ensure_backbone_ws(ut_handle h, int crops) {
  const size_t big = 48 * 48 * 32, small = 24 * 24 * 64;
  return regrow(h, &h->ws_crops, crops, {{&h->bufX, big}, {&h->bufH, big}, {&h->bufY, big}, {&h->bufD, small}});
}

constexpr int PHASE_B_MAX = 8192;

int ensure_phase_b_ws(ut_handle h, int crops) {
  const size_t l2 = 24 * 24 * 64, l3 = 12 * 12 * 128;
  return regrow(h, &h->wsb_crops, crops, {{&h->bufL2, l2}, {&h->bufP, l3}, {&h->bufQ, l3}, {&h->bufBH, l3}, {&h->bufBD, l3}});
}

int ensure_head_ws(ut_handle h, int samples, int n_skel) {
  ut::HeadBuffers& b = h->hb;
  const size_t r = 36 * ut::kRegSplitCh;
  int rc = regrow(h, &h->ws_samples, samples, {{&b.cat144, 36 * 144}, {&b.f108, 36 * 108}, {&b.f72a, 36 * 72}, {&b.f72b, 36 * 72},
                                                {&b.fused, 36 * 72}, {&b.t92a, 36 * 92}, {&b.t92b, 36 * 92}, {&b.regin, r},
                                                {&b.rega, r}, {&b.regb, r}});
  return rc ? rc : regrow(h, &h->ws_skel, n_skel, {{&b.skel, 36 * 4}});
}

int ensure_slots(ut_handle h, int slots, hipStream_t s) {
  if (slots <= h->slots_cap) return UT_OK;
  int cap = h->slots_cap ? h->slots_cap : 2;
  while (cap < slots) cap *= 2;
  float *nm = nullptr, *ne = nullptr, *seen = nullptr;
  int rc;
  if ((rc = dev_alloc(h, &nm, (size_t)cap * 36 * 18)) || (rc = dev_alloc(h, &ne, (size_t)cap * 16)) ||
      (rc = dev_alloc(h, &seen, (size_t)cap)))
    return rc;
  HIPCHK(h, hipMemsetAsync(nm, 0, (size_t)cap * 36 * 18 * sizeof(float), s));
  HIPCHK(h, hipMemsetAsync(ne, 0, (size_t)cap * 16 * sizeof(float), s));
  if (h->slots_cap) {
    HIPCHK(h, hipMemcpyAsync(nm, h->mem, (size_t)h->slots_cap * 36 * 18 * sizeof(float), hipMemcpyDeviceToDevice, s));
    HIPCHK(h, hipMemcpyAsync(ne, h->prev_ext, (size_t)h->slots_cap * 16 * sizeof(float), hipMemcpyDeviceToDevice, s));
    HIPCHK(h, hipStreamSynchronize(s));
    dev_free(h, h->mem);
    dev_free(h, h->prev_ext);
    dev_free(h, h->slot_seen);
  }
  h->mem = nm; h->prev_ext = ne; h->slot_seen = (int*)seen; h->slots_cap = cap;
  return UT_OK;
}

constexpr int kMaxCounters = 4096;
constexpr int kScaleTensors = 33;
static_assert(kScaleTensors < 63, "the adaptation counter is the last of the 64 words at ut_context::calib");
constexpr int kCalibHeadroom = 4;

int begin_call(ut_handle h, hipStream_t s) {
  h->counter_next = 0;
  ++h->word_gen;
  HIPCHK(h, ut::launch_zero_words(h->counters, 2 * kMaxCounters, s));
  return UT_OK;
}

int next_launch_word(ut_handle h, hipStream_t s, int* idx, bool* recycled = nullptr) {
  const bool full = h->counter_next >= kMaxCounters;
  if (full) {
    int rc0 = begin_call(h, s);
    if (rc0) return rc0;
  }
  if (recycled) *recycled = full;
  *idx = h->counter_next++;
  return UT_OK;
}

struct ScaleRef { const unsigned* word = nullptr; const unsigned* obs = nullptr; int adaptive = 0; unsigned* adapt_count = nullptr; };
ScaleRef scale_for(ut_handle h, int tid, const unsigned* producer_word) {
  ScaleRef r;
  if (!h->call_split || h->latency_mode || tid < 0 || tid >= kScaleTensors) return r;
  if (h->calibrating || h->scale_mode == UT_SPLIT_SCALE_DYNAMIC) r.word = producer_word;
  else { r.word = h->calib + tid; r.obs = producer_word; }
  if (!h->calibrating && h->scale_mode == UT_SPLIT_SCALE_CALIBRATED_ADAPTIVE && r.obs) { r.adaptive = 1; r.adapt_count = h->adapt_count; }
  return r;
}
template <class Launch>
int bracket_launch(ut_handle h, hipStream_t s, int in_tid, const unsigned* in_max, double flops, int kind, const char* what,
                   Launch launch) {
  if (h->calibrating && in_max && in_tid >= 0 && in_tid < kScaleTensors) HIPCHK(h, ut::launch_merge_max(h->calib + in_tid, in_max, s));
  ProfEvent pe{nullptr, nullptr, flops, kind};
  if (h->profiling) {
    HIPCHK(h, hipEventCreateWithFlags(&pe.a, hipEventDisableSystemFence));
    HIPCHK(h, hipEventCreateWithFlags(&pe.b, hipEventDisableSystemFence));
    HIPCHK(h, hipEventRecord(pe.a, s));
  }
  const hipError_t e = launch();
  if (e != hipSuccess) return fail(h, UT_E_HIP, what, e);
  if (h->profiling) {
    HIPCHK(h, hipEventRecord(pe.b, s));
    h->prof.push_back(pe);
  }
  return UT_OK;
}

int run_conv(ut_handle h, const ConvW& cw, const float* in, const float* res, float* out, int n_img, int H, int W,
             bool relu, bool nchw, hipStream_t s, const unsigned* in_max = nullptr, unsigned** out_max = nullptr, int in_tid = -1) {
  if (out_max) *out_max = nullptr;
  ut::ConvLaunch c{};
  c.in = in; c.w = cw.w; c.bias = cw.bias; c.res = res; c.out = out;
  c.n_img = n_img; c.H = H; c.W = W; c.cin = cw.cin_pad;
  c.Ho = (H + 2 * cw.pad - cw.ksize) / cw.stride + 1;
  c.Wo = (W + 2 * cw.pad - cw.ksize) / cw.stride + 1;
  c.cout_store = cw.cout_store; c.cout_pad = cw.cout_pad;
  c.k_total = cw.k_total; c.k_pad = cw.k_pad; c.cslice = cw.cslice;
  c.ksize = cw.ksize; c.stride = cw.stride; c.pad = cw.pad;
  c.relu = relu; c.out_nchw = nchw;
  c.device = h->device; c.num_cu = h->num_cu; { static const int kMask[7] = {15, 0, 14, 9, 12, 13, 8}; c.no_resident = kMask[h->resident_weights]; }
  int word = 0;
  bool recycled = false;
  int rc = next_launch_word(h, s, &word, &recycled);
  if (rc) return rc;
  if (recycled) in_max = nullptr;
  c.tile_counter = h->counters + word;
  int splits = 1;
  if (h->latency_mode && !nchw && cw.cout_store % 4 == 0) {
    const long m = (long)n_img * c.Ho * c.Wo;
    const long tiles64 = ((m + 63) / 64) * ((cw.cout_store + 63) / 64);
    const int chunks = cw.k_pad / 32;
    for (int sp = 2; sp <= chunks / 6; ++sp)
      if (chunks % sp == 0 && tiles64 * sp <= (long)h->num_cu && (size_t)sp * m * cw.cout_store <= h->splitk_floats) splits = sp;
  }
  if (h->latency_mode) c.splits = 1;
  if (splits > 1) {
    ut::ConvLaunch part = c;
    part.bias = h->zero_bias; part.res = nullptr; part.relu = 0; part.out = h->splitk_ws; part.splits = splits;
    HIPCHK(h, ut::launch_conv_igemm(part, s));
    HIPCHK(h, ut::launch_splitk_finish(h->splitk_ws, splits, n_img * c.Ho * c.Wo, cw.cout_store, cw.bias, res, out,
                                       relu ? 1 : 0, s));
    return UT_OK;
  }
  const ScaleRef sr = scale_for(h, in_tid, in_max);
  c.w_split = sr.word ? cw.w_split : nullptr;
  c.split_unscale = cw.split_unscale;
  c.status = h->status;
  c.in_max = sr.word;
  c.in_obs = sr.obs;
  c.split_adaptive = sr.adaptive;
  c.adapt_count = sr.adapt_count;
  const int kind = c.w_split && (ut::conv_split_applicable(c) || ut::conv_patch_applicable(c)) ? 1 : 0;
  if (kind) {
    c.out_max = h->counters + kMaxCounters + word;
    if (out_max) *out_max = c.out_max;
  }
  const bool split = c.w_split && ut::conv_split_applicable(c);
  return bracket_launch(h, s, kind ? in_tid : -1, in_max, cw.flops_per_pixel * (double)n_img * c.Ho * c.Wo, kind,
                        split ? "launch_conv_split" : "launch_conv_igemm",
                        [&] { return split ? ut::launch_conv_split(c, s) : ut::launch_conv_igemm(c, s); });
}

int run_block(ut_handle h, const Block& b, const float* x, float* tmp, float* dsbuf, float* y, int n_img, int H,
              int W, hipStream_t s, const unsigned* x_max = nullptr, unsigned** y_max = nullptr, int x_tid = -1, int mid_tid = -1) {
  int rc;
  if (y_max) *y_max = nullptr;
  if (h->counter_next + 8 > kMaxCounters) {
    if ((rc = begin_call(h, s))) return rc;
    x_max = nullptr;
  }
  const ScaleRef xs = scale_for(h, x_tid, x_max);
  if (h->block_fusion && xs.word && !b.has_ds && b.conv1.w_split && b.conv2.w_split && b.conv1.stride == 1 &&
      b.conv1.cin_pad == 32 && b.conv1.cout_store == 32 && b.conv2.cout_store == 32) {
    ut::BlockLaunch bl{};
    bl.in = x; bl.out = y; bl.w1_split = b.conv1.w_split; bl.w2_split = b.conv2.w_split;
    bl.unscale_w1 = b.conv1.split_unscale; bl.unscale_w2 = b.conv2.split_unscale;
    bl.bias1 = b.conv1.bias; bl.bias2 = b.conv2.bias;
    bl.wsum1 = b.conv1.wsum_rows; bl.bmax1 = b.conv1.bias_max;
    bl.in_max = xs.word; bl.in_obs = xs.obs; bl.split_adaptive = xs.adaptive; bl.adapt_count = xs.adapt_count; bl.status = h->status;
    bl.n_img = n_img; bl.H = H; bl.W = W; bl.device = h->device; bl.num_cu = h->num_cu;
    if (ut::conv_block32_applicable((bl.tile_counter = h->counters, bl))) {
      int word = 0;
      bool recycled = false;
      if ((rc = next_launch_word(h, s, &word, &recycled))) return rc;
      if (!recycled) {
        bl.tile_counter = h->counters + word;
        bl.out_max = h->counters + kMaxCounters + word;
        const double flops = (b.conv1.flops_per_pixel + b.conv2.flops_per_pixel) * (double)n_img * H * W;
        if ((rc = bracket_launch(h, s, x_tid, x_max, flops, 1, "launch_conv_block32", [&] { return ut::launch_conv_block32(bl, s); })))
          return rc;
        if (y_max) *y_max = bl.out_max;
        return UT_OK;
      }
    }
  }
  if (h->block_fusion && xs.word && b.has_ds && b.conv1.w_split && b.ds.w_split && b.conv2.w_split &&
      b.conv1.stride == 2 && b.conv1.cin_pad == 32 && b.conv1.cout_store == 64 && b.ds.cout_store == 64 && dsbuf) {
    ut::Stride2Launch sl{};
    sl.in = x; sl.out1 = tmp; sl.out2 = dsbuf; sl.w1_split = b.conv1.w_split; sl.wd_split = b.ds.w_split;
    sl.unscale1 = b.conv1.split_unscale; sl.unscale_d = b.ds.split_unscale;
    sl.bias1 = b.conv1.bias; sl.bias_d = b.ds.bias;
    sl.in_max = xs.word; sl.in_obs = xs.obs; sl.split_adaptive = xs.adaptive; sl.adapt_count = xs.adapt_count; sl.status = h->status;
    sl.n_img = n_img; sl.H = H; sl.W = W; sl.device = h->device; sl.num_cu = h->num_cu;
    if (ut::conv_c32s2_applicable(sl)) {
      int word = 0;
      bool recycled = false;
      if ((rc = next_launch_word(h, s, &word, &recycled))) return rc;
      if (!recycled) {
        sl.out1_max = h->counters + kMaxCounters + word;
        const double flops = (b.conv1.flops_per_pixel + b.ds.flops_per_pixel) * (double)n_img * (H / 2) * (W / 2);
        if ((rc = bracket_launch(h, s, x_tid, x_max, flops, 1, "launch_conv_c32s2", [&] { return ut::launch_conv_c32s2(sl, s); })))
          return rc;
        return run_conv(h, b.conv2, tmp, dsbuf, y, n_img, H / 2, W / 2, true, false, s, sl.out1_max, y_max, mid_tid);
      }
    }
  }
  unsigned* tmp_max = nullptr;
  if ((rc = run_conv(h, b.conv1, x, nullptr, tmp, n_img, H, W, true, false, s, x_max, &tmp_max, x_tid))) return rc;
  const int Ho = (H + 2 - 3) / b.conv1.stride + 1, Wo = (W + 2 - 3) / b.conv1.stride + 1;
  const float* res = x;
  if (b.has_ds) {
    if ((rc = run_conv(h, b.ds, x, nullptr, dsbuf, n_img, H, W, false, false, s))) return rc;
    res = dsbuf;
  }
  return run_conv(h, b.conv2, tmp, res, y, n_img, Ho, Wo, true, false, s, tmp_max, y_max, mid_tid);
}

void prof_clear(ut_handle h) {
  for (auto& pe : h->prof) { (void)hipEventDestroy(pe.a); (void)hipEventDestroy(pe.b); }
  h->prof.clear();
}

int prof_reduce(ut_handle h, hipStream_t s, double ms[2], int64_t launches[2], double flops[2]) {
  h->profiling = false;
  HIPCHK(h, hipStreamSynchronize(s));
  for (int k = 0; k < 2; ++k) { ms[k] = 0; launches[k] = 0; flops[k] = 0; }
  for (auto& pe : h->prof) {
    float t = 0;
    HIPCHK(h, hipEventElapsedTime(&t, pe.a, pe.b));
    const int k = pe.kind ? 1 : 0;
    ms[k] += t; flops[k] += pe.flops; launches[k] += 1;
  }
  prof_clear(h);
  return UT_OK;
}

}

extern "C" {

size_t ut_weight_blob_floats(void) { return UT_WEIGHT_BLOB_FLOATS; }

const char* ut_last_error(ut_handle h) { return h ? h->err.c_str() : g_create_error.c_str(); }

int ut_canonical_backbone_weights(const float* blob, size_t n_floats, float* out, size_t out_floats, size_t* n_out) {
  if (!blob || !n_out) return fail(nullptr, UT_E_INVALID, "ut_canonical_backbone_weights: null argument");
  if (n_floats != UT_WEIGHT_BLOB_FLOATS) return fail(nullptr, UT_E_WEIGHTS, "ut_canonical_backbone_weights: weight blob has the wrong length");
  ut::FoldedNetwork net;
  if (!ut::fold_network(blob, n_floats, net)) return fail(nullptr, UT_E_WEIGHTS, "weight blob length does not match the architecture");
  const ut::FoldedBackbone& fbb = net.backbone;
  std::vector<const ut::Folded*> all = {&fbb.stem};
  for (const ut::FoldedBlock& b : fbb.fb) {
    all.push_back(&b.conv1); all.push_back(&b.conv2);
    if (b.has_ds) all.push_back(&b.ds);
  }
  all.push_back(&fbb.proj);
  size_t n = 0;
  for (const ut::Folded* f : all) n += f->w.size() + f->b.size();
  *n_out = n;
  if (!out) return UT_OK;
  if (out_floats < n) return fail(nullptr, UT_E_INVALID, "ut_canonical_backbone_weights: output too small");
  for (const ut::Folded* f : all) {
    memcpy(out, f->w.data(), f->w.size() * sizeof(float)); out += f->w.size();
    memcpy(out, f->b.data(), f->b.size() * sizeof(float)); out += f->b.size();
  }
  return UT_OK;
}

int ut_create(int device, const float* blob, size_t n_floats, ut_handle* out) {
  if (!blob || !out) return fail(nullptr, UT_E_INVALID, "ut_create: null argument");
  if (n_floats != UT_WEIGHT_BLOB_FLOATS) return fail(nullptr, UT_E_WEIGHTS, "ut_create: weight blob has the wrong length");
  ut::FoldedNetwork net;
  if (!ut::fold_network(blob, n_floats, net)) return fail(nullptr, UT_E_WEIGHTS, "weight blob length does not match the architecture");
  DeviceScope scope(device);
  if (scope.err != hipSuccess) return fail(nullptr, UT_E_HIP, "hipSetDevice", scope.err);
  ut_handle h = new ut_context();
  h->device = device;
  {
    int cus = 0;
    if (hipDeviceGetAttribute(&cus, hipDeviceAttributeMultiprocessorCount, device) == hipSuccess && cus > 0) h->num_cu = cus;
  }
  int rc = UT_OK;
  do {
    { float* cnt = nullptr; if ((rc = dev_alloc(h, &cnt, 2 * kMaxCounters + 64))) break; h->counters = (unsigned*)cnt;
      h->calib = h->counters + 2 * kMaxCounters;
      h->adapt_count = h->calib + 63;
      hipError_t e1 = hipMemset(h->calib, 0, 64 * sizeof(unsigned));
      if (e1 != hipSuccess) { rc = fail(h, UT_E_HIP, "calibration words", e1); break; } }
    { float* st = nullptr; if ((rc = dev_alloc(h, &st, 2))) break; h->status = (int*)st;
      hipError_t e2 = hipMemset(h->status, 0, 2 * sizeof(int));
      if (e2 == hipSuccess) e2 = hipHostMalloc((void**)&h->status_host, 2 * sizeof(int), hipHostMallocDefault);
      if (e2 != hipSuccess) { rc = fail(h, UT_E_HIP, "status words", e2); break; } }
    const ut::FoldedBackbone& fbb = net.backbone;
    if ((rc = upload(h, fbb.stem.w, &h->stem_w)) || (rc = upload(h, fbb.stem.b, &h->stem_b))) break;
    for (int b = 0; b < 12 && !rc; ++b) rc = upload_block(h, h->bb[b], fbb.fb[b]);
    if (rc) break;
    if ((rc = upload_conv(h, h->proj, ut::pack_conv_host(fbb.proj, 1, 1, 72)))) break;
    if ((rc = upload_conv(h, h->fus0, ut::pack_conv_host(net.fusion[0], 1, 1, 108))) ||
        (rc = upload_conv(h, h->fus1, ut::pack_conv_host(net.fusion[1], 1, 1, 72))) ||
        (rc = upload_conv(h, h->fus2, ut::pack_conv_host(net.fusion[2], 1, 1, 72)))) break;
    for (int i = 0; i < 3 && !rc; ++i) rc = upload_conv(h, h->tmp[i], ut::pack_conv_host(net.temporal[i], 1, 1, 92));
    if (rc) break;
    if ((rc = upload(h, net.skel_w, &h->skel_w)) || (rc = upload(h, net.skel_b, &h->skel_b)) ||
        (rc = upload(h, net.skel_scale, &h->skel_scale)) || (rc = upload(h, net.skel_shift, &h->skel_shift))) break;
    if ((rc = upload_regressor(h, h->reg_k, net.reg_k))) break;
    rc = upload_regressor(h, h->reg_u, net.reg_u);
  } while (0);
  if (rc) {
    g_create_error = h->err;
    ut_destroy(h);
    return rc;
  }
  *out = h;
  return UT_OK;
}

int ut_destroy(ut_handle h) {
  if (!h) return UT_OK;
  DeviceScope scope(h->device);
  (void)hipDeviceSynchronize();
  for (void* p : h->allocs) (void)hipFree(p);
  if (h->status_host) (void)hipHostFree(h->status_host);
  for (int i = 0; i < 2; ++i) {
    if (h->lane_stream[i]) (void)hipStreamDestroy(h->lane_stream[i]);
    if (h->ev_join[i]) (void)hipEventDestroy(h->ev_join[i]);
  }
  if (h->ev_fork) (void)hipEventDestroy(h->ev_fork);
  prof_clear(h);
  delete h;
  return UT_OK;
}

int ut_set_backbone_chunk(ut_handle h, int crops_per_pass) {
  if (!h || crops_per_pass < 0) return fail(h, UT_E_INVALID, "ut_set_backbone_chunk: bad argument");
  if (crops_per_pass > kMaxChunk) return fail(h, UT_E_INVALID, "ut_set_backbone_chunk: at most 7281 crops per pass (32-bit offsets)");
  h->chunk = crops_per_pass == 0 ? kDefaultChunk : crops_per_pass;
  return UT_OK;
}

int ut_reserve(ut_handle h, int max_crops, int max_samples, int max_slots) {
  if (!h) return UT_E_INVALID;
  ON_DEVICE_OF(h);
  int rc;
  int c = max_crops < h->chunk ? max_crops : h->chunk;
  if (c > 0 && (rc = ensure_backbone_ws(h, c))) return rc;
  int cb = max_crops < PHASE_B_MAX ? max_crops : PHASE_B_MAX;
  if (cb > 0 && (rc = ensure_phase_b_ws(h, cb))) return rc;
  if (max_samples > 0 && (rc = ensure_head_ws(h, max_samples, max_samples))) return rc;
  if (max_slots > 0 && (rc = ensure_slots(h, max_slots, 0))) return rc;
  if (max_crops > 0 && (rc = regrow(h, &h->crops_ws_floats, (size_t)max_crops * 96 * 96, {{&h->crops_ws, 1}}))) return rc;
  return UT_OK;
}

int ut_warp_crops(ut_handle h, const uint8_t* src, int n_src_images, int src_h, int src_w, const double* cam_params,
                  const double* crop_params, const int32_t* src_index, int n_crops, int remap_mode, float* out,
                  void* stream) {
  if (n_crops == 0) return UT_OK;
  if (!src || !cam_params || !crop_params || !src_index || !out || n_crops < 0 || src_h <= 0 || src_w <= 0 ||
      n_src_images <= 0 || (remap_mode != UT_REMAP_CV2_FIXED && remap_mode != UT_REMAP_FLOAT))
    return fail(h, UT_E_INVALID, "ut_warp_crops: bad argument");
  hipStream_t s = (hipStream_t)stream;
  int *st_dev = nullptr, *st_host = nullptr, mode = UT_CHECK_SYNC, dev = 0;
  if (h) { st_dev = h->status; st_host = h->status_host; mode = h->check_mode; dev = h->device; }
  else {
    DevStatus st;
    int rc = stateless_status(&dev, &st);
    if (rc) return rc;
    st_dev = st.dev; st_host = st.host;
  }
  DeviceScope scope(dev);
  if (scope.err != hipSuccess) return fail(h, UT_E_HIP, "hipSetDevice", scope.err);
  HIPCHK(h, ut::launch_warp(src, n_src_images, src_h, src_w, cam_params, crop_params, src_index, n_crops, remap_mode,
                            out, nullptr, st_dev, s));
  return mode == UT_CHECK_SYNC ? check_status(h, st_dev, st_host, s, "ut_warp_crops") : UT_OK;
}

extern "C" int ut_warp_map(const double* cam_params, const double* crop_params, const int32_t* src_index, int n_src_images,
                           int n_crops, float* out_map, void* stream) {
  if (n_crops == 0) return UT_OK;
  if (!cam_params || !crop_params || !src_index || !out_map || n_crops < 0 || n_src_images <= 0)
    return fail(nullptr, UT_E_INVALID, "ut_warp_map: bad argument");
  HIPCHK(nullptr, ut::launch_warp_map(cam_params, crop_params, src_index, n_src_images, n_crops, out_map, (hipStream_t)stream));
  return UT_OK;
}

static int run_stem(ut_handle h, const float* crops, const uint8_t* crops_u8, float* out, int n, hipStream_t st,
                    unsigned** out_max) {
  *out_max = nullptr;
  if (h->call_split && !h->latency_mode) {
    int word = 0, rc = next_launch_word(h, st, &word);
    if (rc) return rc;
    *out_max = h->counters + kMaxCounters + word;
  }
  if (crops_u8) HIPCHK(h, ut::launch_stem_u8(crops_u8, h->stem_w, h->stem_b, out, n, *out_max, st));
  else HIPCHK(h, ut::launch_stem(crops, h->stem_w, h->stem_b, out, n, *out_max, st));
  return UT_OK;
}

static int backbone_pass(ut_handle h, const float* crops, const uint8_t* crops_u8, float* feat, int c0, int n, int off,
                         int chunk, hipStream_t s) {
  int rc;
  const size_t a48 = (size_t)off * 48 * 48 * 32, a24 = (size_t)off * 24 * 24 * 64, a12 = (size_t)off * 12 * 12 * 128;
  if (h->counter_next + 256 > kMaxCounters && (rc = begin_call(h, s))) return rc;
  unsigned* l2_max = nullptr;
  const unsigned l2_gen = h->word_gen;
  for (int done = 0; done < n; done += chunk) {
    const int m = n - done < chunk ? n - done : chunk;
    const size_t first = (size_t)(c0 + done) * 96 * 96;
    unsigned* xm = nullptr;
    if ((rc = run_stem(h, crops ? crops + first : nullptr, crops_u8 ? crops_u8 + first : nullptr, h->bufX + a48, m, s, &xm))) return rc;
    float *x = h->bufX + a48, *y = h->bufY + a48;
    int hw = 48;
    for (int b = 0; b < 5; ++b) {
      float* dst = b == 4 ? h->bufL2 + a24 + (size_t)done * 24 * 24 * 64 : y;
      if ((rc = run_block(h, h->bb[b], x, h->bufH + a48, h->bufD + a24, dst, m, hw, hw, s, xm, &xm, 2 * b, 2 * b + 1))) return rc;
      hw = (hw + 2 - 3) / h->bb[b].conv1.stride + 1;
      float* t = x; x = y; y = t;
    }
    if (done == 0) l2_max = xm;
    else if (l2_max && xm) HIPCHK(h, ut::launch_merge_max(l2_max, xm, s));
    else l2_max = nullptr;
  }
  const float* x = h->bufL2 + a24;
  float *y = h->bufP + a12, *other = h->bufQ + a12;
  int hw = 24;
  unsigned* xm = l2_gen == h->word_gen ? l2_max : nullptr;
  for (int b = 5; b < 12; ++b) {
    if ((rc = run_block(h, h->bb[b], x, h->bufBH + a12, h->bufBD + a12, y, n, hw, hw, s, xm, &xm, 2 * b, 2 * b + 1))) return rc;
    hw = (hw + 2 - 3) / h->bb[b].conv1.stride + 1;
    x = y;
    float* t = y; y = other; other = t;
  }
  return run_conv(h, h->proj, x, nullptr, feat + (size_t)c0 * 72 * 36, n, 6, 6, false, true, s);
}

static int run_backbone(ut_handle h, const float* crops, const uint8_t* crops_u8, int n_crops, float* feat, hipStream_t s) {
  int rc;
  const int chunk = n_crops < h->chunk ? n_crops : h->chunk;
  if ((rc = ensure_backbone_ws(h, chunk))) return rc;
  const int pass_b = n_crops < PHASE_B_MAX ? n_crops : PHASE_B_MAX;
  if ((rc = ensure_phase_b_ws(h, pass_b))) return rc;
  if ((rc = begin_call(h, s))) return rc;
  h->call_split = h->conv_arith == UT_CONV_SPLIT_F16_ALWAYS || (h->conv_arith == UT_CONV_SPLIT_F16 && n_crops >= 2 * h->num_cu);
  if (h->lanes == 2 && !h->profiling && n_crops <= chunk && n_crops <= pass_b && n_crops >= 1024) {
    if (!h->lane_stream[0]) {
      for (int i = 0; i < 2; ++i) {
        HIPCHK(h, hipStreamCreateWithFlags(&h->lane_stream[i], hipStreamNonBlocking));
        HIPCHK(h, hipEventCreateWithFlags(&h->ev_join[i], hipEventDisableTiming));
      }
      HIPCHK(h, hipEventCreateWithFlags(&h->ev_fork, hipEventDisableTiming));
    }
    HIPCHK(h, hipEventRecord(h->ev_fork, s));
    const int n0 = n_crops / 2;
    for (int i = 0; i < 2; ++i) {
      const int off = i ? n0 : 0, n = i ? n_crops - n0 : n0;
      HIPCHK(h, hipStreamWaitEvent(h->lane_stream[i], h->ev_fork, 0));
      if ((rc = backbone_pass(h, crops, crops_u8, feat, off, n, off, chunk, h->lane_stream[i]))) return rc;
      HIPCHK(h, hipEventRecord(h->ev_join[i], h->lane_stream[i]));
    }
    for (int i = 0; i < 2; ++i) HIPCHK(h, hipStreamWaitEvent(s, h->ev_join[i], 0));
    return UT_OK;
  }
  for (int base = 0; base < n_crops; base += pass_b) {
    const int nb = n_crops - base < pass_b ? n_crops - base : pass_b;
    if ((rc = backbone_pass(h, crops, crops_u8, feat, base, nb, 0, chunk, s))) return rc;
  }
  return UT_OK;
}

static int run_head(ut_handle h, const ut::HeadArgs& a, const float* skel, int n_skel, int mode, float* out_pose, float* out_raw,
                    hipStream_t s);

static int calibrate_head(ut_handle h, const float* feat, int n_crops, hipStream_t s) {
  const int S = n_crops / 2;
  int rc = ensure_head_ws(h, S, 1);
  if (rc) return rc;
  const size_t nf = (size_t)2 * S * 25 + 132 + (size_t)S * (648 + 16 + 60 + 64);
  const size_t off_i64 = (nf * 4 + 7) / 8 * 8, off_i32 = off_i64 + (size_t)4 * S * 8, off_u8 = off_i32 + (size_t)S * 4, total = off_u8 + S;
  std::vector<char> host(total, 0);
  float* f = reinterpret_cast<float*>(host.data());
  for (int c = 0; c < 2 * S; ++c) {
    float* k = f + (size_t)c * 9;
    k[0] = k[4] = 130.f; k[2] = k[5] = 47.5f; k[8] = 1.f;
    float* x = f + (size_t)2 * S * 9 + (size_t)c * 16;
    x[0] = x[5] = x[10] = x[15] = 1.f;
    if (c & 1) x[3] = 0.06f;
  }
  long long* i64 = reinterpret_cast<long long*>(host.data() + off_i64);
  for (int k = 0; k < S; ++k) { i64[2 * k] = 2 * k; i64[2 * k + 1] = 2 * k + 2; i64[2 * S + k] = k; i64[3 * S + k] = k & 1; }
  void* dv = nullptr;
  HIPCHK(h, hipMalloc(&dv, total));
  hipError_t e = hipMemcpyAsync(dv, host.data(), total, hipMemcpyHostToDevice, s);
  if (e == hipSuccess) e = hipStreamSynchronize(s);
  if (e != hipSuccess) { (void)hipFree(dv); return fail(h, UT_E_HIP, "calibration descriptors", e); }
  char* d = static_cast<char*>(dv);
  float* df = reinterpret_cast<float*>(d);
  ut::HeadArgs a{};
  a.feat = feat; a.intrinsics = df; a.extrinsics = df + (size_t)2 * S * 9;
  const float* skel = df + (size_t)2 * S * 25;
  a.mem = df + (size_t)2 * S * 25 + 132; a.prev_ext = a.mem + (size_t)S * 648;
  float* pose = a.prev_ext + (size_t)S * 16;
  float* raw = pose + (size_t)S * 60;
  a.sample_range = reinterpret_cast<const int64_t*>(d + off_i64); a.memory_idx = a.sample_range + 2 * S; a.hand_idx = a.memory_idx + S;
  a.slot_seen = reinterpret_cast<int*>(d + off_i32); a.use_memory = reinterpret_cast<const uint8_t*>(d + off_u8);
  a.n_samples = S; a.n_crops = 2 * S; a.n_slots = S; a.status = h->status; a.call_error_mask = 0;
  rc = begin_call(h, s);
  for (int mode = 0; mode < 2 && !rc; ++mode) rc = run_head(h, a, skel, 1, mode == 0 ? UT_MODE_KNOWN_SKELETON : UT_MODE_UNKNOWN_SKELETON, pose, raw, s);
  (void)hipStreamSynchronize(s);
  (void)hipFree(dv);
  return rc;
}

static int calibrate_split(ut_handle h, const float* crops, int n, hipStream_t s) {
// ... 631 lines not shown
```

absolutetrack_amd/csrc/ut_kernels.h:

```cpp
#pragma once
#include <hip/hip_runtime.h>
#include <stdint.h>

#include "ut_split_pack.h"

namespace ut {

struct ConvLaunch {
  const float* in;
  const float* w;
  const void* w_split;
  float split_unscale;
  int* status;
  const unsigned* in_max;
  const unsigned* in_obs;
  int split_adaptive;
  unsigned* adapt_count;
  unsigned* out_max;
  const float* bias;
  const float* res;
  float* out;
  int n_img, H, W, cin, Ho, Wo;
  int cout_store;
  int cout_pad;
  int k_total;
  int cslice;
  int k_pad;
  int ksize, stride, pad;
  int relu;
  int out_nchw;
  int device;
  int num_cu;
  unsigned* tile_counter;
  int no_resident;
  int splits;
};

hipError_t launch_conv_igemm(const ConvLaunch& c, hipStream_t s);
hipError_t launch_splitk_finish(const float* slabs, int n_splits, int m, int cout_store, const float* bias,
                                const float* res, float* out, int relu, hipStream_t s);
bool conv_split_applicable(const ConvLaunch& c);
hipError_t launch_conv_split(const ConvLaunch& c, hipStream_t s);
struct Stride2Launch {
  const float* in;
  float* out1;
  float* out2;
  const void* w1_split;
  const void* wd_split;
  float unscale1, unscale_d;
  const float* bias1;
  const float* bias_d;
  const unsigned* in_max;
  const unsigned* in_obs;
  int split_adaptive;
  unsigned* adapt_count;
  unsigned* out1_max;
  int* status;
  int n_img, H, W;
  int device, num_cu;
};
bool conv_c32s2_applicable(const Stride2Launch& c);
hipError_t launch_conv_c32s2(const Stride2Launch& c, hipStream_t s);
bool conv_w4_applicable(const ConvLaunch& c);
hipError_t launch_conv_w4(const ConvLaunch& c, hipStream_t s);
bool conv_c64k_applicable(const ConvLaunch& c);
hipError_t launch_conv_c64k(const ConvLaunch& c, hipStream_t s);
struct BlockLaunch {
  const float* in;
  float* out;
  const void* w1_split;
  const void* w2_split;
  float unscale_w1, unscale_w2;
  const float* bias1;
  const float* bias2;
  float wsum1;
  float bmax1;
  const unsigned* in_max;
  const unsigned* in_obs;
  int split_adaptive;
  unsigned* adapt_count;
  unsigned* out_max;
  int* status;
  unsigned* tile_counter;
  int n_img, H, W, device, num_cu;
};
bool conv_block32_applicable(const BlockLaunch& b);
hipError_t launch_conv_block32(const BlockLaunch& b, hipStream_t s);

hipError_t launch_zero_words(void* p, size_t n_words, hipStream_t s);
hipError_t launch_merge_max(unsigned* dst, const unsigned* src, hipStream_t s);
hipError_t launch_raise_words(unsigned* words, int n, int add_exp, hipStream_t s);
hipError_t launch_calibration_crops(float* crops, int n, hipStream_t s);
bool conv_patch_applicable(const ConvLaunch& c);
hipError_t launch_conv_patch(const ConvLaunch& c, hipStream_t s);

hipError_t launch_stem(const float* crops, const float* w , const float* bias ,
                       float* out, int n, unsigned* out_max, hipStream_t s);
hipError_t launch_stem_u8(const uint8_t* crops, const float* w, const float* bias, float* out, int n, unsigned* out_max,
                          hipStream_t s);

struct HeadBuffers {
  float* cat144;
  float* f108;
  float* f72a;
  float* f72b;
  float* fused;
  float* t92a;
  float* t92b;
  float* regin;
  float* rega;
  float* regb;
  float* skel;
  float* xf;
};

enum : int {
  UT_BAD_SAMPLE_RANGE = 1,
  UT_BAD_MEMORY_IDX = 2,
  UT_DUP_MEMORY_IDX = 4,
  UT_BAD_HAND_IDX = 8,
  UT_SINGLE_VIEW = 16,
  UT_BAD_SRC_INDEX = 32,
  UT_SPLIT_RANGE = 64,
};
constexpr int UT_STATUS_ERRORS = UT_BAD_SAMPLE_RANGE | UT_BAD_MEMORY_IDX | UT_DUP_MEMORY_IDX | UT_BAD_HAND_IDX | UT_BAD_SRC_INDEX | UT_SPLIT_RANGE;

#if defined(__HIPCC__)
__device__ __forceinline__ unsigned abs_bits(float v) { return __float_as_uint(v) & 0x7FFFFFFFu; }

__device__ __forceinline__ void publish_abs_max(unsigned* word, unsigned lane_bits) {
#pragma unroll
  for (int o = 32; o; o >>= 1) {
    const unsigned other = (unsigned)__shfl_xor((int)lane_bits, o);
    lane_bits = other > lane_bits ? other : lane_bits;
  }
  if ((threadIdx.x & 63) == 0 && lane_bits > __hip_atomic_load(word, __ATOMIC_RELAXED, __HIP_MEMORY_SCOPE_AGENT))
    atomicMax(word, lane_bits);
}

__device__ __forceinline__ int split_pow2_for(int e, bool none, float& scale, float& unscale) {
  int k = none ? 0 : 141 - e;
  k = k > 100 ? 100 : k < -100 ? -100 : k;
  scale = __uint_as_float((unsigned)(127 + k) << 23);
  unscale = __uint_as_float((unsigned)(127 - k) << 23);
  return k;
}

__device__ __forceinline__ unsigned split_act_scale(const unsigned* in_max, const unsigned* in_obs, bool adaptive, float& scale,
                                                    float& unscale, bool& ok, bool& adapted) {
  unsigned bits = (unsigned)__builtin_amdgcn_readfirstlane((int)*in_max);
  const unsigned obs = in_obs ? (unsigned)__builtin_amdgcn_readfirstlane((int)*in_obs) : 0u;
  const int eo = (int)(obs >> 23);
  int e = (int)(bits >> 23);
  int k = split_pow2_for(e, bits == 0u || e == 255, scale, unscale);
  adapted = adaptive && in_obs && obs != 0u && eo != 255 && (eo + k > 142 || eo + 11 < e);
  if (adapted) {
    bits = obs;
    e = eo;
    k = split_pow2_for(e, false, scale, unscale);
  }
  ok = e != 255;
  if (in_obs && !adapted && (eo == 255 || eo + k > 142)) ok = false;
  return bits;
}

__device__ __forceinline__ void split_scale_report(bool ok, bool adapted, int* status, unsigned* adapt_count) {
  if (threadIdx.x == 0 && blockIdx.x == 0) {
    if (!ok && status) atomicOr(status, UT_SPLIT_RANGE);
    if (adapted && adapt_count) atomicAdd(adapt_count, 1u);
  }
}
#endif

struct HeadArgs {
  const float* feat;
  const float* intrinsics;
  const float* extrinsics;
  const int64_t* sample_range;
  const int64_t* memory_idx;
  const uint8_t* use_memory;
  const int64_t* hand_idx;
  int n_samples;
  int n_crops;
  int n_slots;
  float* mem;
  float* prev_ext;
  int* status;
  int call_error_mask;
  int* slot_seen;
};

hipError_t launch_validate_desc(const HeadArgs& a, hipStream_t s);

hipError_t launch_ftl_in(const HeadArgs& a, const HeadBuffers& b, hipStream_t s);
hipError_t launch_ftl_out_temporal_in(const HeadArgs& a, const HeadBuffers& b, hipStream_t s);
hipError_t launch_temporal_out(const HeadArgs& a, const float* t_out , const float* skel,
                               int n_skel, float* regin, int reg_c, int reg_stride, unsigned* out_max, hipStream_t s);
hipError_t launch_skeleton(const float* skel_in , const float* w ,
                           const float* bias , const float* bn_scale ,
                           const float* bn_shift , float* out , int n_skel,
                           hipStream_t s);
hipError_t launch_pool_decode(const HeadArgs& a, const float* reg_feat , int reg_c, int reg_stride,
                              const float* w , const float* bias , int d,
                              float* out_pose, float* out_raw, float* raw_ws , hipStream_t s);

hipError_t launch_fk(const float* hand_model, int n_models, const float* ja, int ja_stride,
                     const float* xf, int xf_stride, const int64_t* mirror, float t_scale, int n,
                     float* out, hipStream_t s);

constexpr int MESH_MAX_VERTICES = 5056;
hipError_t launch_skin_mesh(const float* hand_model, int n_models, const float* ja, int ja_stride, const float* xf,
                            int xf_stride, const int64_t* mirror, float t_scale, int n, const void* verts,
                            const uint32_t* csr_off, const uint32_t* csr_ent, int nv, float* out_v, float* out_n,
                            hipStream_t s);

enum : int { PROJECT_FISHEYE62 = 0, PROJECT_PINHOLE = 1 };
struct ProjectArgs {
  const float* points;
  int point_stride, n_points;
  const int32_t* cam_rows;
  int max_views;
  const double* table;
  int n_rows, kind, n;
  int width, height;
  double* window;
  double* eye_z;
  uint8_t* flags;
  int* status;
};
hipError_t launch_project_points(const ProjectArgs& g, hipStream_t s);

constexpr int RENDER_CROP = 96;
constexpr int RENDER_MAX_VERTICES = 2368;
struct RenderArgs {
  const float* vertices;
  int nv;
  const int4* tris;
  int nt;
  const double* crop_params;
  const int64_t* sample_range;
  int n, n_crops;
  float* depth;
  int32_t* tri;
  uint8_t* shade;
  int* status;
};
hipError_t launch_render_check(const RenderArgs& g, hipStream_t s);
hipError_t launch_render_mesh(const RenderArgs& g, hipStream_t s);

struct CropGenArgs {
  const double* cam_params;
  const double* camera_angles;
  const float* hand_model;
  const float* joint_limits;
  const float* joint_angles;
  const float* wrist_xf;
  const int32_t* frame_idx;
  const int64_t* hand_idx;
  int n, n_models, n_cams, max_views, min_vis, src_w, src_h, crop_size;
  double focal_multiplier;
  double* crop_params;
  float* intrinsics;
  float* extrinsics;
  int32_t* cam_index;
  int32_t* n_views;
  int32_t* status;
  float* landmarks;
};
hipError_t launch_cropgen(const CropGenArgs& g, hipStream_t s);

struct CropGenWindowArgs {
  const double* cam_params;
  const double* keypoints;
  const int32_t* src_row;
  const int64_t* hand_idx;
  int n, max_views, crop_size;
  double focal_multiplier;
  double* crop_params;
  float* intrinsics;
  float* extrinsics;
  int32_t* cam_index;
  int32_t* n_views;
  int32_t* status;
};
hipError_t launch_cropgen_window(const CropGenWindowArgs& g, hipStream_t s);

struct CropMatArgs {
  const float* orig_extrinsics;
  const float* orig_intrinsics;
  const float* crop_points;
  const int64_t* hand_idx;
  int n_frames, n_views, n_pts, crop_size;
  double focal_multiplier;
  float* extrinsics_xf;
  float* new_intrinsics;
  float* resample_xf;
  int32_t* status;
};
hipError_t launch_cropmat(const CropMatArgs& g, hipStream_t s);
hipError_t launch_resample_homography(const void* src, int src_is_f32, int n, int src_h, int src_w,
                                      const float* resample_xf, int out_h, int out_w, float* out, hipStream_t s);

hipError_t launch_keypoint_metrics(const float* gt, const float* tracked, const uint8_t* valid, int n_hands, int n_frames,
                                   double* err, double* acc, double* gt_acc, uint8_t* valid_acc, hipStream_t s);

hipError_t launch_mem_export(const float* mem , float* out , int slots, hipStream_t s);

hipError_t launch_warp(const uint8_t* src, int n_src, int src_h, int src_w, const double* cam,
                       const double* crop, const int32_t* src_index, int n_crops, int mode, float* out,
                       uint8_t* out_u8, int* status, hipStream_t s);

hipError_t launch_warp_map(const double* cam, const double* crop, const int32_t* src_index, int n_src, int n_crops,
                           float* out, hipStream_t s);

}
```

absolutetrack_amd/csrc/ut_split_pack.h:

```cpp
#pragma once
#include <stddef.h>
#include <stdint.h>

namespace ut {

size_t pack_split_weights(const float* w, int cout_pad, int k_pad, float scale, uint16_t* out);
float split_weight_scale(const float* w, size_t n);

}
```

absolutetrack_amd/csrc/ut_weights.cpp:

```cpp
#include "ut_weights.h"

#include <math.h>

#include "ut_split_pack.h"

namespace ut {
namespace {

struct Cursor {
  const float* p;
  size_t left;
  const float* take(size_t n) {
    if (n > left) { left = 0; ok = false; return nullptr; }
    const float* r = p; p += n; left -= n; return r;
  }
  bool ok = true;
};

struct BN { const float *g = nullptr, *b = nullptr, *m = nullptr, *v = nullptr; };

BN take_bn(Cursor& c, int ch) {
  BN bn;
  bn.g = c.take(ch); bn.b = c.take(ch); bn.m = c.take(ch); bn.v = c.take(ch);
  c.take(1);
  return bn;
}

Folded fold_conv(const float* w, const float* conv_bias, const BN* bn, int cin, int cout, int taps) {
  Folded f;
  f.cin = cin; f.cout = cout; f.taps = taps;
  f.w.resize((size_t)cout * cin * taps);
  f.b.resize(cout);
  for (int o = 0; o < cout; ++o) {
    double s = 1.0, shift = conv_bias ? (double)conv_bias[o] : 0.0;
    if (bn) {
      s = (double)bn->g[o] / sqrt((double)bn->v[o] + 1e-5);
      shift = (shift - (double)bn->m[o]) * s + (double)bn->b[o];
    }
    f.b[o] = (float)shift;
    for (size_t i = (size_t)o * cin * taps; i < (size_t)(o + 1) * cin * taps; ++i) f.w[i] = (float)((double)w[i] * s);
  }
  return f;
}

float row_max(const Folded& f, int o) {
  float m = fabsf(f.b[o]);
  const size_t n = (size_t)f.cin * f.taps;
  for (size_t i = 0; i < n; ++i) {
    const float a = fabsf(f.w[(size_t)o * n + i]);
    m = a > m ? a : m;
  }
  return m;
}
int octave_shift(float m) {
  if (!(m > 0.f) || !(m < INFINITY)) return 0;
  return -ilogbf(m);
}
void scale_row(Folded& f, int o, int k) {
  if (!k) return;
  const size_t n = (size_t)f.cin * f.taps;
  for (size_t i = 0; i < n; ++i) f.w[(size_t)o * n + i] = ldexpf(f.w[(size_t)o * n + i], k);
  f.b[o] = ldexpf(f.b[o], k);
}
void scale_col(Folded& f, int c, int k) {
  if (!k) return;
  for (int o = 0; o < f.cout; ++o)
    for (int t = 0; t < f.taps; ++t) {
      float& v = f.w[((size_t)o * f.cin + c) * f.taps + t];
      v = ldexpf(v, k);
    }
}
void canonicalise_channels(const std::vector<Folded*>& keys, const std::vector<Folded*>& producers,
                           const std::vector<Folded*>& consumers) {
  const int ch = keys[0]->cout;
  for (int c = 0; c < ch; ++c) {
    float m = 0.f;
    for (Folded* p : keys) { const float r = row_max(*p, c); m = r > m ? r : m; }
    const int k = octave_shift(m);
    for (Folded* p : producers) scale_row(*p, c, k);
    for (Folded* q : consumers) scale_col(*q, c, -k);
  }
}

Folded pad_channels(const Folded& f, int cin, int cout) {
  Folded g;
  g.cin = cin; g.cout = cout; g.taps = f.taps;
  g.w.assign((size_t)cout * cin * f.taps, 0.f);
  g.b.assign(cout, 0.f);
  for (int o = 0; o < f.cout; ++o) {
    g.b[o] = f.b[o];
    for (int c = 0; c < f.cin; ++c)
      for (int t = 0; t < f.taps; ++t) g.w[((size_t)o * cin + c) * f.taps + t] = f.w[((size_t)o * f.cin + c) * f.taps + t];
  }
  return g;
}

bool fold_block(Cursor& c, FoldedBlock& fb, int cin, int cout, int stride, bool ds) {
  const float* w1 = c.take((size_t)cout * cin * 9);
  BN bn1 = take_bn(c, cout);
  const float* w2 = c.take((size_t)cout * cout * 9);
  BN bn2 = take_bn(c, cout);
  const float* wd = nullptr;
  BN bnd;
  if (ds) { wd = c.take((size_t)cout * cin); bnd = take_bn(c, cout); }
  if (!c.ok) return false;
  fb.stride = stride; fb.has_ds = ds;
  fb.conv1 = fold_conv(w1, nullptr, &bn1, cin, cout, 9);
  fb.conv2 = fold_conv(w2, nullptr, &bn2, cout, cout, 9);
  if (ds) fb.ds = fold_conv(wd, nullptr, &bnd, cin, cout, 1);
  return true;
}

void canonicalise_inner(FoldedBlock& fb) { canonicalise_channels({&fb.conv1}, {&fb.conv1}, {&fb.conv2}); }

bool fold_backbone(Cursor& c, FoldedBackbone& out) {
  const float* sw = c.take(32 * 9);
  const float* sb = c.take(32);
  BN sbn = take_bn(c, 32);
  if (!c.ok) return false;
  Folded& stem = out.stem;
  Folded& proj = out.proj;
  FoldedBlock* fb = out.fb;
  stem = fold_conv(sw, sb, &sbn, 1, 32, 9);
  const int nb[4] = {2, 3, 5, 2}, planes[4] = {32, 64, 128, 256}, strides[4] = {1, 2, 2, 2};
  int first_of_layer[5] = {0, 0, 0, 0, 12};
  int cin = 32, bi = 0;
  for (int l = 0; l < 4; ++l) {
    first_of_layer[l] = bi;
    for (int k = 0; k < nb[l]; ++k) {
      int st = k == 0 ? strides[l] : 1;
      bool ds = k == 0 && (st != 1 || cin != planes[l]);
      if (!fold_block(c, fb[bi++], cin, planes[l], st, ds)) return false;
      cin = planes[l];
    }
  }
  const float* pw = c.take(72 * 256); const float* pb = c.take(72);
  if (!c.ok) return false;
  proj = fold_conv(pw, pb, nullptr, 256, 72, 1);
  for (int l = 0; l < 4; ++l) {
    const int b0 = first_of_layer[l], b1 = l < 3 ? first_of_layer[l + 1] : 12;
    std::vector<Folded*> keys, prod, cons;
    if (fb[b0].has_ds) {
      canonicalise_inner(fb[b0]);
      keys = {&fb[b0].ds, &fb[b0].conv2};
      prod = {&fb[b0].ds};
    } else {
      keys = {&stem};
      prod = {&stem};
      cons.push_back(&fb[b0].conv1);
    }
    for (int b = b0; b < b1; ++b) {
      prod.push_back(&fb[b].conv2);
      if (b > b0) cons.push_back(&fb[b].conv1);
    }
    if (l < 3) { cons.push_back(&fb[b1].conv1); cons.push_back(&fb[b1].ds); }
    else cons.push_back(&proj);
    canonicalise_channels(keys, prod, cons);
    for (int b = fb[b0].has_ds ? b0 + 1 : b0; b < b1; ++b) canonicalise_inner(fb[b]);
  }
  return true;
}

bool fold_regressor(Cursor& c, FoldedRegressor& r, int ch, int d) {
  r.c = ch; r.d = d;
  for (int i = 0; i < 2; ++i) {
    FoldedBlock& fb = r.blocks[i];
    if (!fold_block(c, fb, ch, ch, 1, false)) return false;
    canonicalise_inner(fb);
    r.wide[i].conv1 = pad_channels(fb.conv1, kRegSplitCh, kRegSplitCh);
    r.wide[i].conv2 = pad_channels(fb.conv2, kRegSplitCh, kRegSplitCh);
  }
  const float* w = c.take((size_t)d * ch);
  const float* b = c.take(d);
  if (!c.ok) return false;
  r.w_out.assign(w, w + (size_t)d * ch);
  r.b_out.assign(b, b + d);
  return true;
}

}

bool fold_network(const float* blob, size_t n, FoldedNetwork& out) {
  Cursor c{blob, n};
  if (!fold_backbone(c, out.backbone)) return false;
  const float* w0 = c.take(108 * 144); const float* b0 = c.take(108); BN bn0 = take_bn(c, 108);
  const float* w1 = c.take(72 * 108); const float* b1 = c.take(72); BN bn1 = take_bn(c, 72);
  const float* w2 = c.take(72 * 72); const float* b2 = c.take(72);
  const float *tw[3], *tb[3];
  for (int i = 0; i < 3; ++i) { tw[i] = c.take(90 * 90); tb[i] = c.take(90); }
  const float* lw = c.take(144 * 132); const float* lb = c.take(144); BN bn = take_bn(c, 4);
  if (!c.ok) return false;
  out.fusion[0] = fold_conv(w0, b0, &bn0, 144, 108, 1);
  out.fusion[1] = fold_conv(w1, b1, &bn1, 108, 72, 1);
  out.fusion[2] = fold_conv(w2, b2, nullptr, 72, 72, 1);
  for (int i = 0; i < 3; ++i) out.temporal[i] = fold_conv(tw[i], tb[i], nullptr, 90, 90, 1);
  out.skel_w.assign(lw, lw + 144 * 132);
  out.skel_b.assign(lb, lb + 144);
  out.skel_scale.resize(4); out.skel_shift.resize(4);
  for (int k = 0; k < 4; ++k) {
    double s = (double)bn.g[k] / sqrt((double)bn.v[k] + 1e-5);
    out.skel_scale[k] = (float)s; out.skel_shift[k] = (float)((double)bn.b[k] - (double)bn.m[k] * s);
  }
  return fold_regressor(c, out.reg_k, 76, 62) && fold_regressor(c, out.reg_u, 72, 63) && c.left == 0;
}

PackedConv pack_conv_host(const Folded& f, int ksize, int stride, int cout_store) {
  PackedConv cw;
  const int cin = f.cin, cout = f.cout;
  cw.cin = cin; cw.cout = cout; cw.ksize = ksize; cw.stride = stride;
  cw.pad = ksize == 3 ? 1 : 0;
  cw.taps = ksize * ksize;
  cw.cin_pad = round_up(cin, 4);
  cw.cout_store = cout_store;
  cw.cout_pad = round_up(cout_store, 128);
  cw.k_total = cw.taps * cw.cin_pad;
  cw.cslice = cw.cin_pad % 32 == 0 ? 32 : cw.cin_pad;
  cw.k_pad = round_up(cw.k_total, 32);
  cw.flops_per_pixel = 2.0 * cw.taps * cin * cout;
  std::vector<float>& wp = cw.wp;
  std::vector<float>& bp = cw.bp;
  wp.assign((size_t)cw.cout_pad * cw.k_pad, 0.f);
  bp.assign(cw.cout_pad, 0.f);
  for (int o = 0; o < cout; ++o) {
    bp[o] = f.b[o];
    for (int c = 0; c < cin; ++c)
      for (int t = 0; t < cw.taps; ++t)
        wp[(size_t)o * cw.k_pad + (c / cw.cslice) * (cw.taps * cw.cslice) + t * cw.cslice + c % cw.cslice] =
            f.w[((size_t)o * cin + c) * cw.taps + t];
  }
  {
    double ws = 0.0, bm = 0.0;
    for (int o = 0; o < cout; ++o) {
      double rs = 0.0;
      for (int k = 0; k < cw.k_pad; ++k) rs += fabs((double)wp[(size_t)o * cw.k_pad + k]);
      ws = rs > ws ? rs : ws;
      bm = fabs((double)bp[o]) > bm ? fabs((double)bp[o]) : bm;
    }
    cw.wsum_rows = (float)(ws * 1.0001);
    cw.bias_max = (float)(bm * 1.0001);
  }
  if (cw.cslice == 32 && (cw.k_pad / 32 >= 6 || (ksize == 1 && stride == 2 && cw.cin_pad == 32)) && cw.cout_store >= 32 && cw.cout_store % 4 == 0) {
    cw.planes.resize((size_t)2 * cw.cout_pad * cw.k_pad);
    const float scale = split_weight_scale(wp.data(), wp.size());
    cw.split_unscale = 1.0f / scale;
    pack_split_weights(wp.data(), cw.cout_pad, cw.k_pad, scale, cw.planes.data());
  }
  return cw;
}

}
```

absolutetrack_amd/csrc/ut_weights.h:

```cpp
#pragma once
#include <stddef.h>
#include <stdint.h>

#include <vector>

namespace ut {

constexpr int kRegSplitCh = 128;

inline int round_up(int v, int m) { return (v + m - 1) / m * m; }

struct Folded {
  std::vector<float> w;
  std::vector<float> b;
  int cin = 0, cout = 0, taps = 0;
};

struct FoldedBlock {
  Folded conv1, conv2, ds;
  bool has_ds = false;
  int stride = 1;
};

struct FoldedBackbone {
  Folded stem, proj;
  FoldedBlock fb[12];
};

struct FoldedRegressor {
  FoldedBlock blocks[2];
  FoldedBlock wide[2];
  std::vector<float> w_out;
  std::vector<float> b_out;
  int c = 0, d = 0;
};

struct FoldedNetwork {
  FoldedBackbone backbone;
  Folded fusion[3];
  Folded temporal[3];
  std::vector<float> skel_w, skel_b;
  std::vector<float> skel_scale, skel_shift;
  FoldedRegressor reg_k, reg_u;
};

bool fold_network(const float* blob, size_t n, FoldedNetwork& out);

struct ConvGeom {
  int cin = 0, cin_pad = 0, cout = 0, cout_pad = 0, cout_store = 0;
  int taps = 1, ksize = 1, stride = 1, pad = 0, k_total = 0, k_pad = 0, cslice = 0;
  double flops_per_pixel = 0;
};

struct PackedConv : ConvGeom {
  std::vector<float> wp;
  std::vector<float> bp;
  std::vector<uint16_t> planes;
  float split_unscale = 0.f;
  float wsum_rows = 0.f;
  float bias_max = 0.f;
};

PackedConv pack_conv_host(const Folded& f, int ksize, int stride, int cout_store);

}
```

Baseline: 167,800 hand-frames/s.

## Fold downsample shortcut 1x1 conv into second conv of stride-2 residual blocks

The 1x1 stride-2 downsample convolution of residual blocks is folded into the following 3x3 conv2 kernel. conv2 gains a pre-phase that reads the block input at stride 2, applies the split-fp16 shortcut weights into the same accumulators, rescales them, and uses a pre-summed bias. The c32s2 fused kernel can now skip its downsample output when the fold is active. This removes the dsbuf write and read plus a separate launch, at the cost of extra kernel complexity and a rescaling step that could affect precision.

```diff
diff --git a/absolutetrack_amd/csrc/conv_c32s2.hip b/absolutetrack_amd/csrc/conv_c32s2.hip
--- a/absolutetrack_amd/csrc/conv_c32s2.hip
+++ b/absolutetrack_amd/csrc/conv_c32s2.hip
@@ -41,10 +41,11 @@
     split_scale_report(ok, adapted, p.status, p.adapt_count);
   }
   const float unscale1 = p.unscale1 * x_unscale, unscale_d = p.unscale_d * x_unscale;
+  const bool has_d = __builtin_amdgcn_readfirstlane(p.out2 != nullptr ? 1 : 0) != 0;
 
   const u32x4 a_words = rsrc_words(p.in, (unsigned)((size_t)M_in * CIN * sizeof(float)));
   const __amdgpu_buffer_rsrc_t o1_rsrc = __builtin_amdgcn_make_buffer_rsrc(p.out1, 0, (int)((size_t)M_out * COUT * sizeof(float)), 0x00020000);
-  const __amdgpu_buffer_rsrc_t o2_rsrc = __builtin_amdgcn_make_buffer_rsrc(p.out2, 0, (int)((size_t)M_out * COUT * sizeof(float)), 0x00020000);
+  const __amdgpu_buffer_rsrc_t o2_rsrc = __builtin_amdgcn_make_buffer_rsrc(p.out2 ? p.out2 : p.out1, 0, has_d ? (int)((size_t)M_out * COUT * sizeof(float)) : 0, 0x00020000);
 
   u32x4 wa[32], wd[4];
   {
@@ -96,9 +97,13 @@
       for (int q = 0; q < 4; ++q)
         *reinterpret_cast<u32x4*>(smem + S_W8 + cb * 4096 + q * 1024 + lane * 16) = *reinterpret_cast<const u32x4*>(wg + 8 * 4096 + q * 1024);
     }
-    const char* dg = reinterpret_cast<const char*>(p.wd_split) + (size_t)cb * 4096 + lane * 16;
-#pragma unroll
-    for (int q = 0; q < 4; ++q) wd[q] = *reinterpret_cast<const u32x4*>(dg + q * 1024);
+#pragma unroll
+    for (int q = 0; q < 4; ++q) wd[q] = u32x4{0, 0, 0, 0};
+    if (has_d) {
+      const char* dg = reinterpret_cast<const char*>(p.wd_split) + (size_t)cb * 4096 + lane * 16;
+#pragma unroll
+      for (int q = 0; q < 4; ++q) wd[q] = *reinterpret_cast<const u32x4*>(dg + q * 1024);
+    }
   }
   const unsigned w8 = (unsigned)(S_W8 + cb * 4096 + lane * 16);
 
@@ -169,7 +174,7 @@
   __builtin_amdgcn_s_barrier();
 
   unsigned out_bits = 0;
-  const float bias1 = p.bias1[32 * cb + fr], bias_d = p.bias_d[32 * cb + fr];
+  const float bias1 = p.bias1[32 * cb + fr], bias_d = has_d ? p.bias_d[32 * cb + fr] : 0.f;
   const int o_ = 32 * blk + fr, oy_ = o_ / Wo, ox_ = o_ - oy_ * Wo;
   const int lrow = 2 * oy_ * W + 2 * ox_ - 1;
   const unsigned mask_left = ox_ == 0 ? 0x1FFu & ~0x49u : 0x1FFu;
@@ -228,7 +233,7 @@
     if constexpr ((TAP) < 8) { S_MFMA_A(acc, TAP, S, 0, CUR[0]); }                                   \
     else if constexpr ((S) == 1) { S_MFMA_V_LAST(acc, w8a_, CUR[0]); } else { S_MFMA_V(acc, w8a_, CUR[0]); } \
     S_PIN();                                                                                         \
-    if constexpr ((TAP) == 4) {                     \
+    if constexpr ((TAP) == 4) if (has_d) {          \
       if constexpr ((S) == 0) { S_MFMA_V_FIRST(accd, wd[0], CUR[1]); } else { S_MFMA_V(accd, wd[2], CUR[1]); } \
       S_PIN();                                                                                       \
       S_MFMA_V(accd, wd[2 * (S) + 1], CUR[0]); S_PIN();                                              \
@@ -254,9 +259,11 @@
       __builtin_amdgcn_raw_buffer_store_b32(__float_as_uint(o), o1_rsrc, S_ROFF(off, r), 0, 0);      \
     }                                                                                                \
     out_bits = max(out_bits, mx);                                                                    \
-    _Pragma("unroll") for (int r = 0; r < 16; ++r) {                                                 \
-      const float o = __builtin_fmaf(accd[r], unscale_d, bias_d);                                    \
-      __builtin_amdgcn_raw_buffer_store_b32(__float_as_uint(o), o2_rsrc, S_ROFF(off, r), 0, 0);      \
+    if (has_d) {                                                                                     \
+      _Pragma("unroll") for (int r = 0; r < 16; ++r) {                                               \
+        const float o = __builtin_fmaf(accd[r], unscale_d, bias_d);                                  \
+        __builtin_amdgcn_raw_buffer_store_b32(__float_as_uint(o), o2_rsrc, S_ROFF(off, r), 0, 0);    \
+      }                                                                                              \
     }                                                                                                \
   }
 
@@ -329,7 +336,7 @@
 }
 
 bool conv_c32s2_applicable(const Stride2Launch& c) {
-  return c.in && c.out1 && c.out2 && c.w1_split && c.wd_split && c.unscale1 > 0.f && c.unscale_d > 0.f && c.in_max && c.W == 48 &&
+  return c.in && c.out1 && c.w1_split && (!c.out2 || (c.wd_split && c.bias_d && c.unscale_d > 0.f)) && c.unscale1 > 0.f && c.in_max && c.W == 48 &&
          c.H % 8 == 0 && c.H >= 8 && c.n_img > 0 && c.num_cu > 0 && (size_t)c.n_img * c.H * c.W * 32 * sizeof(float) < 0x7FFFFF00ull;
 }
 
diff --git a/absolutetrack_amd/csrc/conv_split.hip b/absolutetrack_amd/csrc/conv_split.hip
--- a/absolutetrack_amd/csrc/conv_split.hip
+++ b/absolutetrack_amd/csrc/conv_split.hip
@@ -576,30 +576,5 @@
   return halo ? launch_split_cfg<256, 128, 4, 2, true>(c, s) : launch_split_cfg<256, 128, 4, 2, false>(c, s);
 }
 
-size_t pack_split_weights(const float* w, int cout_pad, int k_pad, float scale, uint16_t* out) {
-  const int n_chunks = k_pad / 32;
-  for (int grp = 0; grp < cout_pad / 32; ++grp)
-    for (int kc = 0; kc < n_chunks; ++kc)
-      for (int st = 0; st < 2; ++st)
-        for (int ln = 0; ln < 64; ++ln)
-          for (int e = 0; e < 8; ++e) {
-            const float x = w[(size_t)(grp * 32 + (ln & 31)) * k_pad + kc * 32 + 16 * st + 8 * (ln >> 5) + e] * scale;
-            const _Float16 h0 = (_Float16)x;
-            const _Float16 h1 = (_Float16)(x - (float)h0);
-            const size_t base = ((((size_t)grp * n_chunks + kc) * 2 + st) * 2) * 512 + (size_t)ln * 8 + e;
-            __builtin_memcpy(&out[base], &h0, 2);
-            __builtin_memcpy(&out[base + 512], &h1, 2);
-          }
-  return (size_t)2 * cout_pad * k_pad;
-}
-
-float split_weight_scale(const float* w, size_t n) {
-  float m = 0.f;
-  for (size_t i = 0; i < n; ++i) m = fmaxf(m, fabsf(w[i]));
-  if (!(m > 0.f) || !(m < 3.0e38f)) return 1.f;
-  int e;
-  frexpf(m, &e);
-  return ldexpf(1.f, 15 - e);
-}
-
-}
+
+}
diff --git a/absolutetrack_amd/csrc/conv_w4.hip b/absolutetrack_amd/csrc/conv_w4.hip
--- a/absolutetrack_amd/csrc/conv_w4.hip
+++ b/absolutetrack_amd/csrc/conv_w4.hip
@@ -14,11 +14,12 @@
 static_assert(9 % W4_NSET == 0, "the register sets of the weight fragments line up across slices");
 constexpr int w4_cap(int pixels, int wi, int hi) { return ((pixels / (wi * hi)) * (hi + 1) * (wi + 1) + 2 * (wi + 2) + 15) / 16 * 16; }
 
-template <int WI, int HI, int SCH, int WPX, bool S2 = false>
+template <int WI, int HI, int SCH, int WPX, bool S2 = false, bool SC = false>
 __global__ __launch_bounds__(256, 1) void conv_w4_kernel(ConvLaunch p, int tiles_n, int n_tiles) {
   extern __shared__ __attribute__((aligned(16))) char smem[];
   constexpr int MI = W4_MI, PW = WI + 1, PH = HI + 1, HW = WI * HI;
   static_assert(!S2 || (SCH == 32 && WPX == 1), "phase planes: two 16-channel planes per buffer, four 32-channel blocks per tile");
+  static_assert(!SC || !S2, "shortcut pre-phase: SCH-channel passes through the patch buffer the first slice begins rewriting");
   constexpr int BM = W4_WPIX * WPX;
   constexpr int NCB = 4 / WPX, BN = 32 * NCB;
   constexpr int NG = SCH / 4, NHG = NG / 2;
@@ -57,9 +58,21 @@
   const __amdgpu_buffer_rsrc_t q_rsrc = __builtin_amdgcn_make_buffer_rsrc(p.tile_counter, 0, 4, 0x00020000);
 
   float x_scale = 1.f, x_unscale = 1.f;
+  [[maybe_unused]] float sc_scale = 1.f, sc_ratio = 1.f;
   if (p.in_max) {
     bool ok, adapted;
     split_act_scale(p.in_max, p.in_obs, p.split_adaptive, x_scale, x_unscale, ok, adapted);
+    if constexpr (SC) {
+      float sc_unscale;
+      bool ok2, adapted2;
+      split_act_scale(p.sc_max, p.sc_obs, p.sc_adaptive, sc_scale, sc_unscale, ok2, adapted2);
+      const auto ex = [](float f) { return (int)((__float_as_uint(f) >> 23) & 255u); };
+      int r = ex(x_scale) - ex(p.split_unscale) - ex(sc_scale) + ex(p.sc_unscale);
+      ok = ok && ok2 && r >= -64 && r <= 64;
+      adapted = adapted || adapted2;
+      r = r > 64 ? 64 : r < -64 ? -64 : r;
+      sc_ratio = __uint_as_float((unsigned)(127 + r) << 23);
+    }
     split_scale_report(ok, adapted, p.status, p.adapt_count);
   }
   const float tot_unscale = p.split_unscale * x_unscale;
@@ -127,11 +140,12 @@
   }
 #define W4_PIN() { __builtin_amdgcn_sched_barrier(0); asm volatile("" ::: "memory"); __builtin_amdgcn_sched_barrier(0); }
 #define W4_ROW_OFF(I, R) ((unsigned)((I) * 32 + 8 * ((R) >> 2) + ((R) & 3)) * row_bs)
-#define W4_SPLIT_STORE(V, WA)                                                                        \
+#define W4_SPLIT_STORE(V, WA) W4_SPLIT_STORE_S(V, WA, x_scale)
+#define W4_SPLIT_STORE_S(V, WA, SCL)                                                                 \
   {                                                                                                  \
     unsigned a0_, b0_, a1_, b1_;                                                                     \
-    split_pair_scaled((V).x, (V).y, x_scale, a0_, b0_);                                              \
-    split_pair_scaled((V).z, (V).w, x_scale, a1_, b1_);                                              \
+    split_pair_scaled((V).x, (V).y, SCL, a0_, b0_);                                                  \
+    split_pair_scaled((V).z, (V).w, SCL, a1_, b1_);                                                  \
     *reinterpret_cast<u32x2*>(smem + (WA)) = u32x2{a0_, a1_};                                        \
     *reinterpret_cast<u32x2*>(smem + (WA) + NHG * GSTRIDE) = u32x2{b0_, b1_};                        \
   }
@@ -316,7 +330,70 @@
         const unsigned row_after = last_slice ? w_row_next : w_row;
         W4S_SLICE()
       }
-    } else
+    } else {
+    if constexpr (SC) {
+      constexpr int SKS = SCH / 16;
+      const int n_sc = p.sc_cin / SCH;
+      const int n_sch = p.sc_cin / 32;
+      const __amdgpu_buffer_rsrc_t s_rsrc = __builtin_amdgcn_make_buffer_rsrc(
+          const_cast<float*>(p.sc_in), 0, (int)((size_t)M * 4 * p.sc_cin * sizeof(float)), 0x00020000);
+      const __amdgpu_buffer_rsrc_t sw_rsrc = __builtin_amdgcn_make_buffer_rsrc(
+          const_cast<void*>(p.sc_w_split), 0, (int)((size_t)(p.cout_pad / 32) * n_sch * 4096), 0x00020000);
+      const unsigned sbuf = (unsigned)__builtin_amdgcn_readfirstlane(((cur_buf + NBUF - 1) % NBUF) * STAGE);
+      const unsigned cbuf = (unsigned)__builtin_amdgcn_readfirstlane(cur_buf * STAGE);
+      const unsigned s_tb = (unsigned)((tile / tiles_n) * (BM * 4)) * (unsigned)p.sc_cin * 4u;
+      const unsigned s_wrow = (unsigned)(((tile % tiles_n) * NCB + wco) * n_sch) * 4096u;
+      float4 sv[W4_NLOAD];
+      unsigned sb[MI];
+#pragma unroll
+      for (int i = 0; i < MI; ++i) sb[i] = pb[i] + sbuf;
+#define W4_SC_LOAD(PASS)                                                                             \
+      _Pragma("unroll") for (int j = 0; j < W4_NLOAD; ++j) {                                         \
+        const int k = RP * j + tid / NG, img = k / HW, rem = k - img * HW, y = rem / WI, x = rem - y * WI; \
+        const unsigned o_ = (unsigned)(((img * 2 * HI + 2 * y) * 2 * WI + 2 * x) * p.sc_cin + 4 * (tid % NG)) * 4u; \
+        sv[j] = __builtin_bit_cast(float4, __builtin_amdgcn_raw_buffer_load_b128(s_rsrc, s_tb + o_, (unsigned)(PASS) * (SCH * 4u), 0)); \
+      }
+      W4_SC_LOAD(0)
+      for (int ps = 0; ps < n_sc; ++ps) {
+        u32x4 sw[SKS][2];
+        const unsigned s_woff = s_wrow + (unsigned)(SKS == 2 ? ps * 4096 : (ps >> 1) * 4096 + (ps & 1) * 2048);
+#pragma unroll
+        for (int f = 0; f < 2 * SKS; ++f)
+          sw[f >> 1][f & 1] = __builtin_bit_cast(u32x4, __builtin_amdgcn_raw_buffer_load_b128(sw_rsrc, w_lane, s_woff + (unsigned)(f * 1024), 0));
+#pragma unroll
+        for (int j = 0; j < W4_NLOAD; ++j) W4_SPLIT_STORE_S(sv[j], sbuf + h_wa[j], sc_scale)
+        __syncthreads();
+        if (ps + 1 < n_sc) { W4_SC_LOAD(ps + 1) }
+#pragma unroll
+        for (int st = 0; st < SKS; ++st) {
+#pragma unroll
+          for (int i = 0; i < MI; ++i) {
+            if (st == 0) { W4_READ_X(i, 1, 0, 4, sb) W4_READ_X(i, 0, 0, 4, sb) }
+            else { W4_READ_X(i, 1, 1, 4, sb) W4_READ_X(i, 0, 1, 4, sb) }
+          }
+#pragma unroll
+          for (int n = 0; n < 3 * MI; ++n) {
+            const int pr = n / MI, i = n % MI;
+            acc[i] = __builtin_amdgcn_mfma_f32_32x32x16_f16(__builtin_bit_cast(f16x8, xp[i][pr == 0 ? 1 : 0]),
+                                                            __builtin_bit_cast(f16x8, sw[st][pr == 1 ? 1 : 0]), acc[i], 0, 0, 0);
+          }
+        }
+        __syncthreads();
+      }
+#undef W4_SC_LOAD
+#pragma unroll
+      for (int i = 0; i < MI; ++i)
+#pragma unroll
+        for (int e = 0; e < 16; ++e) acc[i][e] *= sc_ratio;
+      unsigned cb[MI];
+#pragma unroll
+      for (int i = 0; i < MI; ++i) cb[i] = pb[i] + cbuf;
+#pragma unroll
+      for (int i = 0; i < MI; ++i) {
+        W4_READ_X(i, 1, 0, 0, cb)
+        if (i < MI - 1) { W4_READ_X(i, 0, 0, 0, cb) }
+      }
+    }
     for (int sl = 0; sl < n_slices; ++sl) {
       const bool last_slice = sl == n_slices - 1;
       const int b1 = cur_buf + 1 == NBUF ? 0 : cur_buf + 1, b2 = b1 + 1 == NBUF ? 0 : b1 + 1;
@@ -333,6 +410,7 @@
       for (int i = 0; i < MI; ++i) { rb[i] = pb[i] + rbuf; nb[i] = pb[i] + nbuf; }
       W4_SLICE()
       cur_buf = b1;
+    }
     }
     {
       const int tm = tile / tiles_n, tn = tile - tm * tiles_n;
@@ -423,6 +501,7 @@
 #undef W4_PIN
 #undef W4_ROW_OFF
 #undef W4_SPLIT_STORE
+#undef W4_SPLIT_STORE_S
 #undef W4_SLOT_BODY
 #undef W4_SLICE
 #undef W4S_PLANE
@@ -439,7 +518,7 @@
 #undef W4S_SLICE
 }
 
-template <int WI, int HI, int SCH, int WPX, bool S2 = false>
+template <int WI, int HI, int SCH, int WPX, bool S2 = false, bool SC = false>
 hipError_t launch_w4_cfg(const ConvLaunch& c, hipStream_t s) {
   constexpr int BM = W4_WPIX * WPX, BN = 128 / WPX;
   const long M = (long)c.n_img * c.Ho * c.Wo;
@@ -447,11 +526,11 @@
   const int n_tiles = tiles_m * tiles_n;
   constexpr int lds = (SCH == 32 ? 2 : 3) * (SCH / 4) * w4_cap(BM, WI, HI) * 16 + 16 + 4 * 4096;
   static std::atomic<unsigned long long> attr_set{0};
-  const hipError_t attr_e = set_dynamic_lds_once(attr_set, c.device, lds, &conv_w4_kernel<WI, HI, SCH, WPX, S2>);
+  const hipError_t attr_e = set_dynamic_lds_once(attr_set, c.device, lds, &conv_w4_kernel<WI, HI, SCH, WPX, S2, SC>);
   if (attr_e != hipSuccess) return attr_e;
   int grid = c.num_cu;
   if (grid > n_tiles) grid = n_tiles;
-  hipLaunchKernelGGL((conv_w4_kernel<WI, HI, SCH, WPX, S2>), dim3(grid), dim3(256), lds, s, c, tiles_n, n_tiles);
+  hipLaunchKernelGGL((conv_w4_kernel<WI, HI, SCH, WPX, S2, SC>), dim3(grid), dim3(256), lds, s, c, tiles_n, n_tiles);
   return hipGetLastError();
 }
 
@@ -464,6 +543,12 @@
                       (size_t)c.n_img * c.H * c.W * c.cin * sizeof(float) < 0x7FFFFF00ull &&
                       (size_t)c.n_img * c.Ho * c.Wo * c.cout_store * sizeof(float) < 0x7FFFFF00ull;
   if (!common) return false;
+  if (c.sc_in)
+    return c.stride == 1 && c.cin >= 64 && c.H == c.Ho && c.W == c.Wo && !c.res && c.in_max && c.sc_max &&
+           c.sc_w_split && c.sc_unscale > 0.f && c.sc_cin >= 32 && c.sc_cin <= 256 && c.sc_cin % 32 == 0 &&
+           (size_t)c.n_img * 4 * c.H * c.W * c.sc_cin * sizeof(float) < 0x7FFFFF00ull &&
+           (c.cout_store % 128 == 0 ? (c.W == 12 && c.H == 12) || (c.W == 6 && c.H == 6)
+                                    : !(c.no_resident & 4) && c.cout_store == 64 && c.W == 24 && c.H == 24);
   if (c.stride == 2)
     return !(c.no_resident & 8) && c.cin >= 64  && c.cout_store % 128 == 0 && c.H == 2 * c.Ho && c.W == 2 * c.Wo && !c.res &&
            ((c.Wo == 12 && c.Ho == 12) || (c.Wo == 6 && c.Ho == 6));
@@ -475,6 +560,10 @@
 hipError_t launch_conv_w4(const ConvLaunch& c, hipStream_t s) {
   if (!conv_w4_applicable(c)) return hipErrorInvalidValue;
   if (c.stride == 2) return c.Wo == 12 ? launch_w4_cfg<12, 12, 32, 1, true>(c, s) : launch_w4_cfg<6, 6, 32, 1, true>(c, s);
+  if (c.sc_in)
+    return c.W == 24   ? launch_w4_cfg<24, 24, 16, 2, false, true>(c, s)
+           : c.W == 12 ? launch_w4_cfg<12, 12, 32, 1, false, true>(c, s)
+                       : launch_w4_cfg<6, 6, 32, 1, false, true>(c, s);
   if (c.W == 24) return launch_w4_cfg<24, 24, 16, 2>(c, s);
   return c.W == 12 ? launch_w4_cfg<12, 12, 32, 1>(c, s) : launch_w4_cfg<6, 6, 32, 1>(c, s);
 }
diff --git a/absolutetrack_amd/csrc/ut_api.hip b/absolutetrack_amd/csrc/ut_api.hip
--- a/absolutetrack_amd/csrc/ut_api.hip
+++ b/absolutetrack_amd/csrc/ut_api.hip
@@ -26,6 +26,10 @@
   float wsum_rows = 0.f;
   float bias_max = 0.f;
   float* bias = nullptr;
+  void* sc_split = nullptr;
+  float sc_unscale = 0.f;
+  int sc_cin = 0;
+  float* bias_fold = nullptr;
 };
 
 struct Block {
@@ -208,6 +212,11 @@
   cw.split_unscale = pc.split_unscale; cw.wsum_rows = pc.wsum_rows; cw.bias_max = pc.bias_max;
   int rc = upload(h, pc.wp, &cw.w);
   if (!rc && !pc.planes.empty()) rc = upload_bytes(h, pc.planes.data(), pc.planes.size() * sizeof(uint16_t), &cw.w_split);
+  if (!rc && !pc.sc_planes.empty()) {
+    cw.sc_unscale = pc.sc_unscale; cw.sc_cin = pc.sc_cin;
+    rc = upload_bytes(h, pc.sc_planes.data(), pc.sc_planes.size() * sizeof(uint16_t), &cw.sc_split);
+    if (!rc) rc = upload(h, pc.bp_fold, &cw.bias_fold);
+  }
   return rc ? rc : upload(h, pc.bp, &cw.bias);
 }
 
@@ -215,10 +224,15 @@
   int rc;
   const int cs = ut::round_up(fb.conv1.cout, 4);
   if ((rc = upload_conv(h, b.conv1, ut::pack_conv_host(fb.conv1, 3, fb.stride, cs)))) return rc;
-  if ((rc = upload_conv(h, b.conv2, ut::pack_conv_host(fb.conv2, 3, 1, cs)))) return rc;
+  ut::PackedConv conv2 = ut::pack_conv_host(fb.conv2, 3, 1, cs);
   b.has_ds = fb.has_ds;
-  if (fb.has_ds && (rc = upload_conv(h, b.ds, ut::pack_conv_host(fb.ds, 1, fb.stride, cs)))) return rc;
-  return UT_OK;
+  if (fb.has_ds) {
+    const ut::PackedConv ds = ut::pack_conv_host(fb.ds, 1, fb.stride, cs);
+    if ((cs % 128 == 0 || (cs == 64 && ds.cin_pad == 32)) && fb.stride == 2 && !ut::fold_shortcut_host(conv2, ds))
+      return fail(h, UT_E_WEIGHTS, "upload_block: the shortcut of a down-sampling block does not fold into its second convolution");
+    if ((rc = upload_conv(h, b.ds, ds))) return rc;
+  }
+  return upload_conv(h, b.conv2, conv2);
 }
 
 int upload_regressor(ut_handle h, Regressor& r, const ut::FoldedRegressor& fr) {
@@ -352,8 +366,11 @@
   return UT_OK;
 }
 
+struct FoldedShortcut { const float* x; ScaleRef xs; double flops_per_pixel; };
+
 int run_conv(ut_handle h, const ConvW& cw, const float* in, const float* res, float* out, int n_img, int H, int W,
-             bool relu, bool nchw, hipStream_t s, const unsigned* in_max = nullptr, unsigned** out_max = nullptr, int in_tid = -1) {
+             bool relu, bool nchw, hipStream_t s, const unsigned* in_max = nullptr, unsigned** out_max = nullptr, int in_tid = -1,
+             const FoldedShortcut* sc = nullptr) {
   if (out_max) *out_max = nullptr;
   ut::ConvLaunch c{};
   c.in = in; c.w = cw.w; c.bias = cw.bias; c.res = res; c.out = out;
@@ -401,8 +418,16 @@
     c.out_max = h->counters + kMaxCounters + word;
     if (out_max) *out_max = c.out_max;
   }
+  double flops_per_pixel = cw.flops_per_pixel;
+  if (sc) {
+    c.sc_in = sc->x; c.sc_cin = cw.sc_cin; c.sc_max = sc->xs.word; c.sc_obs = sc->xs.obs; c.sc_adaptive = sc->xs.adaptive;
+    c.sc_w_split = cw.sc_split; c.sc_unscale = cw.sc_unscale; c.bias = cw.bias_fold;
+    if (sc->xs.adaptive) { c.adapt_count = sc->xs.adapt_count; }
+    flops_per_pixel += sc->flops_per_pixel;
+    if (!c.w_split || !ut::conv_w4_applicable(c)) return fail(h, UT_E_INVALID, "run_conv: no kernel for a convolution with a folded shortcut");
+  }
   const bool split = c.w_split && ut::conv_split_applicable(c);
-  return bracket_launch(h, s, kind ? in_tid : -1, in_max, cw.flops_per_pixel * (double)n_img * c.Ho * c.Wo, kind,
+  return bracket_launch(h, s, kind ? in_tid : -1, in_max, flops_per_pixel * (double)n_img * c.Ho * c.Wo, kind,
                         split ? "launch_conv_split" : "launch_conv_igemm",
                         [&] { return split ? ut::launch_conv_split(c, s) : ut::launch_conv_igemm(c, s); });
 }
@@ -442,8 +467,9 @@
   }
   if (h->block_fusion && xs.word && b.has_ds && b.conv1.w_split && b.ds.w_split && b.conv2.w_split &&
       b.conv1.stride == 2 && b.conv1.cin_pad == 32 && b.conv1.cout_store == 64 && b.ds.cout_store == 64 && dsbuf) {
+    const bool fold = (h->resident_weights == 1 || h->resident_weights == 6) && b.conv2.sc_split && H == 48 && W == 48;
     ut::Stride2Launch sl{};
-    sl.in = x; sl.out1 = tmp; sl.out2 = dsbuf; sl.w1_split = b.conv1.w_split; sl.wd_split = b.ds.w_split;
+    sl.in = x; sl.out1 = tmp; sl.out2 = fold ? nullptr : dsbuf; sl.w1_split = b.conv1.w_split; sl.wd_split = b.ds.w_split;
     sl.unscale1 = b.conv1.split_unscale; sl.unscale_d = b.ds.split_unscale;
     sl.bias1 = b.conv1.bias; sl.bias_d = b.ds.bias;
     sl.in_max = xs.word; sl.in_obs = xs.obs; sl.split_adaptive = xs.adaptive; sl.adapt_count = xs.adapt_count; sl.status = h->status;
@@ -454,9 +480,13 @@
       if ((rc = next_launch_word(h, s, &word, &recycled))) return rc;
       if (!recycled) {
         sl.out1_max = h->counters + kMaxCounters + word;
-        const double flops = (b.conv1.flops_per_pixel + b.ds.flops_per_pixel) * (double)n_img * (H / 2) * (W / 2);
+        const double flops = (b.conv1.flops_per_pixel + (fold ? 0.0 : b.ds.flops_per_pixel)) * (double)n_img * (H / 2) * (W / 2);
         if ((rc = bracket_launch(h, s, x_tid, x_max, flops, 1, "launch_conv_c32s2", [&] { return ut::launch_conv_c32s2(sl, s); })))
           return rc;
+        if (fold) {
+          const FoldedShortcut sc{x, xs, b.ds.flops_per_pixel};
+          return run_conv(h, b.conv2, tmp, nullptr, y, n_img, H / 2, W / 2, true, false, s, sl.out1_max, y_max, mid_tid, &sc);
+        }
         return run_conv(h, b.conv2, tmp, dsbuf, y, n_img, H / 2, W / 2, true, false, s, sl.out1_max, y_max, mid_tid);
       }
     }
@@ -465,6 +495,11 @@
   if ((rc = run_conv(h, b.conv1, x, nullptr, tmp, n_img, H, W, true, false, s, x_max, &tmp_max, x_tid))) return rc;
   const int Ho = (H + 2 - 3) / b.conv1.stride + 1, Wo = (W + 2 - 3) / b.conv1.stride + 1;
   const float* res = x;
+  if (h->block_fusion && (h->resident_weights == 1 || h->resident_weights == 6) && xs.word && tmp_max && b.has_ds && b.conv2.sc_split &&
+      b.conv1.stride == 2 && ((Ho == 12 && Wo == 12) || (Ho == 6 && Wo == 6)) && H == 2 * Ho && W == 2 * Wo) {
+    const FoldedShortcut sc{x, xs, b.ds.flops_per_pixel};
+    return run_conv(h, b.conv2, tmp, nullptr, y, n_img, Ho, Wo, true, false, s, tmp_max, y_max, mid_tid, &sc);
+  }
   if (b.has_ds) {
     if ((rc = run_conv(h, b.ds, x, nullptr, dsbuf, n_img, H, W, false, false, s))) return rc;
     res = dsbuf;
diff --git a/absolutetrack_amd/csrc/ut_kernels.h b/absolutetrack_amd/csrc/ut_kernels.h
--- a/absolutetrack_amd/csrc/ut_kernels.h
+++ b/absolutetrack_amd/csrc/ut_kernels.h
@@ -33,6 +33,13 @@
   int num_cu;
   unsigned* tile_counter;
   int no_resident;
+  const float* sc_in;
+  int sc_cin;
+  const unsigned* sc_max;
+  const unsigned* sc_obs;
+  int sc_adaptive;
+  const void* sc_w_split;
+  float sc_unscale;
   int splits;
 };
 
diff --git a/absolutetrack_amd/csrc/ut_split_pack.h b/absolutetrack_amd/csrc/ut_split_pack.h
--- a/absolutetrack_amd/csrc/ut_split_pack.h
+++ b/absolutetrack_amd/csrc/ut_split_pack.h
@@ -1,10 +1,34 @@
 #pragma once
+#include <math.h>
 #include <stddef.h>
 #include <stdint.h>
 
 namespace ut {
 
-size_t pack_split_weights(const float* w, int cout_pad, int k_pad, float scale, uint16_t* out);
-float split_weight_scale(const float* w, size_t n);
+inline size_t pack_split_weights(const float* w, int cout_pad, int k_pad, float scale, uint16_t* out) {
+  const int n_chunks = k_pad / 32;
+  for (int grp = 0; grp < cout_pad / 32; ++grp)
+    for (int kc = 0; kc < n_chunks; ++kc)
+      for (int st = 0; st < 2; ++st)
+        for (int ln = 0; ln < 64; ++ln)
+          for (int e = 0; e < 8; ++e) {
+            const float x = w[(size_t)(grp * 32 + (ln & 31)) * k_pad + kc * 32 + 16 * st + 8 * (ln >> 5) + e] * scale;
+            const _Float16 h0 = (_Float16)x;
+            const _Float16 h1 = (_Float16)(x - (float)h0);
+            const size_t base = ((((size_t)grp * n_chunks + kc) * 2 + st) * 2) * 512 + (size_t)ln * 8 + e;
+            __builtin_memcpy(&out[base], &h0, 2);
+            __builtin_memcpy(&out[base + 512], &h1, 2);
+          }
+  return (size_t)2 * cout_pad * k_pad;
+}
+
+inline float split_weight_scale(const float* w, size_t n) {
+  float m = 0.f;
+  for (size_t i = 0; i < n; ++i) m = fmaxf(m, fabsf(w[i]));
+  if (!(m > 0.f) || !(m < 3.0e38f)) return 1.f;
+  int e;
+  frexpf(m, &e);
+  return ldexpf(1.f, 15 - e);
+}
 
 }
diff --git a/absolutetrack_amd/csrc/ut_weights.cpp b/absolutetrack_amd/csrc/ut_weights.cpp
--- a/absolutetrack_amd/csrc/ut_weights.cpp
+++ b/absolutetrack_amd/csrc/ut_weights.cpp
@@ -248,4 +248,18 @@
   return cw;
 }
 
-}
+bool fold_shortcut_host(PackedConv& conv2, const PackedConv& ds) {
+  if (conv2.planes.empty() || conv2.ksize != 3 || conv2.stride != 1 || ds.ksize != 1 || ds.stride != 2 || ds.cslice != 32 ||
+      ds.k_pad != ds.cin_pad || ds.cin_pad % 32 != 0 || ds.cout_pad != conv2.cout_pad || ds.cout_store != conv2.cout_store)
+    return false;
+  const float scale = split_weight_scale(ds.wp.data(), ds.wp.size());
+  conv2.sc_planes.resize((size_t)2 * ds.cout_pad * ds.k_pad);
+  pack_split_weights(ds.wp.data(), ds.cout_pad, ds.k_pad, scale, conv2.sc_planes.data());
+  conv2.sc_unscale = 1.0f / scale;
+  conv2.sc_cin = ds.cin_pad;
+  conv2.bp_fold.resize(conv2.cout_pad);
+  for (int o = 0; o < conv2.cout_pad; ++o) conv2.bp_fold[o] = conv2.bp[o] + ds.bp[o];
+  return true;
+}
+
+}
diff --git a/absolutetrack_amd/csrc/ut_weights.h b/absolutetrack_amd/csrc/ut_weights.h
--- a/absolutetrack_amd/csrc/ut_weights.h
+++ b/absolutetrack_amd/csrc/ut_weights.h
@@ -59,8 +59,13 @@
   float split_unscale = 0.f;
   float wsum_rows = 0.f;
   float bias_max = 0.f;
+  std::vector<uint16_t> sc_planes;
+  std::vector<float> bp_fold;
+  float sc_unscale = 0.f;
+  int sc_cin = 0;
 };
 
 PackedConv pack_conv_host(const Folded& f, int ksize, int stride, int cout_store);
+bool fold_shortcut_host(PackedConv& conv2, const PackedConv& ds);
 
 }
```

Result: faster. 170,800 hand-frames/s (median of 6 runs) (+1.8%).
